# lemerleau/RAFFT

Hardware: AMD Instinct MI355X
Metric: sequences/sec (whole node) on benchmark set, beam N=100; kcal/mol MAE vs CPU (higher is better)
Workload: dtype f32 FFT -> exact int counts, f64 scores, i32 dcal energies

## Files before the change

rafft_amd/csrc/rafft_beam.hip:

```cpp
#pragma once


__device__ inline bool seen_lookup(const uint64_t *tab, uint32_t cap, uint64_t h1, uint64_t h2, uint32_t &free_sl)
{
    const uint32_t mask = cap - 1;
    uint32_t sl = (uint32_t)h1 & mask;
    const ulonglong2 *t2 = (const ulonglong2 *)tab;
    for (;;) {
        const uint32_t s1 = (sl + 1) & mask, s2 = (sl + 2) & mask, s3 = (sl + 3) & mask;
        ulonglong2 e0 = t2[sl], e1 = t2[s1], e2 = t2[s2], e3 = t2[s3];
        pin(e0); pin(e1); pin(e2); pin(e3);
        if (e0.x == 0) { free_sl = sl; return false; }
        if (e0.x == h1 && e0.y == h2) return true;
        if (e1.x == 0) { free_sl = s1; return false; }
        if (e1.x == h1 && e1.y == h2) return true;
        if (e2.x == 0) { free_sl = s2; return false; }
        if (e2.x == h1 && e2.y == h2) return true;
        if (e3.x == 0) { free_sl = s3; return false; }
        if (e3.x == h1 && e3.y == h2) return true;
        sl = (sl + 4) & mask;
    }
}
__device__ inline void seen_insert_at(uint64_t *tab, uint32_t cap, uint64_t h1, uint64_t h2, uint32_t sl)
{
    const uint32_t mask = cap - 1;
    for (;;) {
        unsigned long long old = atomicCAS((unsigned long long *)&tab[2 * (uint64_t)sl], 0ULL, (unsigned long long)h1);
        if (old == 0) { tab[2 * (uint64_t)sl + 1] = h2; return; }
        if (old == h1 && tab[2 * (uint64_t)sl + 1] == h2) return;
        sl = (sl + 1) & mask;
    }
}
__device__ inline bool seen_insert_new(uint64_t *tab, uint32_t cap, uint64_t h1, uint64_t h2)
{
    uint32_t mask = cap - 1, sl = (uint32_t)h1 & mask;
    for (;;) {
        unsigned long long old = atomicCAS((unsigned long long *)&tab[2 * (uint64_t)sl], 0ULL, (unsigned long long)h1);
        if (old == 0) { tab[2 * (uint64_t)sl + 1] = h2; return true; }
        if (old == h1 && tab[2 * (uint64_t)sl + 1] == h2) return false;
        sl = (sl + 1) & mask;
    }
}
__device__ inline void seen_insert(uint64_t *tab, uint32_t cap, uint64_t h1, uint64_t h2)
{
    uint32_t mask = cap - 1, sl = (uint32_t)h1 & mask;
    for (;;) {
        unsigned long long old = atomicCAS((unsigned long long *)&tab[2 * (uint64_t)sl], 0ULL, (unsigned long long)h1);
        if (old == 0) { tab[2 * (uint64_t)sl + 1] = h2; return; }
        if (old == h1 && tab[2 * (uint64_t)sl + 1] == h2) return;
        sl = (sl + 1) & mask;
    }
}


template <int NT>
__device__ inline void seen_rehash(const uint64_t *stab, uint32_t scap, uint64_t *ntab, uint32_t ncap, int tid)
{
    const ulonglong2 *src = (const ulonglong2 *)stab;
    const uint32_t mask = ncap - 1;
    for (uint32_t base = 0; base < scap; base += NT * 4) {
        ulonglong2 e[4];
        unsigned long long old[4];
#pragma unroll
        for (int u = 0; u < 4; u++) { const uint32_t i = base + (uint32_t)u * NT + (uint32_t)tid; e[u] = i < scap ? src[i] : make_ulonglong2(0ULL, 0ULL); }
#pragma unroll
        for (int u = 0; u < 4; u++) { old[u] = 1; if (e[u].x) old[u] = atomicCAS((unsigned long long *)&ntab[2 * (uint64_t)((uint32_t)e[u].x & mask)], 0ULL, (unsigned long long)e[u].x); }
#pragma unroll
        for (int u = 0; u < 4; u++)
            if (e[u].x) {
                if (old[u] == 0) ntab[2 * (uint64_t)((uint32_t)e[u].x & mask) + 1] = e[u].y;
                else seen_insert(ntab, ncap, e[u].x, e[u].y);
            }
    }
}

struct ParentInfo {
    unsigned long long total, cur;
    unsigned long long h1, h2;
    int dcal0, flag;
    int sid, nprod;
    unsigned long long prod;
    int rl0, nrl;
};
static_assert(sizeof(ParentInfo) == 64, "ParentInfo layout");

__device__ __forceinline__ unsigned long long sat_mul(unsigned long long a, unsigned long long b)
{
    const unsigned long long lim = 1ULL << 62;
    if (a == 0 || b == 0) return 0;
    return (a > lim / b) ? lim : a * b;
}

template <int BS_NT>
__global__ __launch_bounds__(BS_NT, BS_NT == 256 ? 5 : 1) void beam_step_kernel(Dev d, int sort_cap)
{
    extern __shared__ __align__(16) unsigned char lds[];
    const size_t r0 = max((size_t)8 * (size_t)sort_cap, (size_t)24 * BS_NT);
    unsigned long long *skey = (unsigned long long *)lds;
    unsigned long long *wk_h1 = (unsigned long long *)lds;
    unsigned long long *wk_h2 = wk_h1 + BS_NT;
    unsigned int *wk_tab = (unsigned int *)(wk_h2 + BS_NT);
    unsigned long long *rl_off = (unsigned long long *)(lds + r0);
    int *rl_cnt = (int *)(rl_off + RL_CAP);
    ParentInfo *pinfo = (ParentInfo *)(rl_cnt + RL_CAP);
    unsigned long long *ppre = (unsigned long long *)(pinfo + d.B);
    int *oldbeam = (int *)(ppre + d.B + 1);
    int *sh = oldbeam + ((d.B + 3) & ~3);
    const int tid = threadIdx.x, lane = tid & 63, wv = tid >> 6;
    const int sq = blockIdx.x;
    if (sq == 0 && tid < NSHARD) d.c->node_prev[tid].v = d.c->node[tid].v;
    if (sq == 0 && tid < NCLS) d.c->n_work[tid].v = 0;
    if (sq == 0) for (int i = tid; i < NCLS * NSHARD; i += BS_NT) d.c->wcur[i / NSHARD][i % NSHARD].v = 0;
    if (sq == 0 && tid < NCLS) d.c->wdone[tid] = 0;
    if (d.done[sq]) return;
    if (tid == 0) sh[27] = d.c->overflow != 0 ? 1 : 0;
    __syncthreads();
    if (sh[27]) return;
    const int nbeam = d.beam_n[sq];
    const int step_no = d.nsteps[sq];
    int *beam = d.beam + (size_t)sq * d.B;
    for (int i = tid; i < nbeam; i += BS_NT) oldbeam[i] = beam[i];
    __syncthreads();

    if (d.traj) {
        if (tid == 0) {
            unsigned long long r = atomicAdd(&d.c->trec_n, 1ULL);
            unsigned long long o = atomicAdd(&d.c->tsid_top, (unsigned long long)nbeam);
            if (r >= d.trec_cap || o + nbeam > d.tsid_cap) { atomicOr(&d.c->overflow, OVF_TRAJ); sh[0] = -1; }
            else { d.trec[r] = make_int4(sq, d.nsteps[sq], nbeam, (int)o); sh[0] = (int)o; }
        }
        __syncthreads();
        int o = sh[0];
        if (o >= 0) for (int i = tid; i < nbeam; i += BS_NT) d.tsid[o + i] = oldbeam[i];
        __syncthreads();
    }
    if (tid == 0) d.nsteps[sq] += 1;

    {
        unsigned long long *istart = ppre;
        int *pnode0 = sh + 32;
        unsigned int irun = 0;
        if (tid == 0) sh[28] = 0;
        __syncthreads();
        for (int b0 = 0; b0 < nbeam; b0 += BS_NT) {
            const int b = b0 + tid;
            int ic = 0;
            if (b < nbeam) {
                const int sid = oldbeam[b];
                StRec r;
                {
                    const uint4 *rp = (const uint4 *)&d.st[sid];
                    uint4 q0 = rp[0], q1 = rp[1], q2 = rp[2], q3 = rp[3], q4 = rp[4], q5 = rp[5], q6 = rp[6];
                    pin(q0); pin(q1); pin(q2); pin(q3); pin(q4); pin(q5); pin(q6);
                    auto u64 = [](unsigned int lo, unsigned int hi) { return (unsigned long long)lo | ((unsigned long long)hi << 32); };
                    r.dcal = (int)q0.y; r.node0 = (int)q0.z; r.nnodes = (int)q0.w; r.nprod = (int)q1.y; r.c0d = (int)q1.z;
                    r.h1 = u64(q2.x, q2.y); r.h2 = u64(q2.z, q2.w); r.cursor = u64(q3.z, q3.w); r.total = u64(q4.z, q4.w);
                    r.prod = u64(q5.x, q5.y); r.c0h1 = u64(q5.z, q5.w); r.c0h2 = u64(q6.x, q6.y);
                }
                ParentInfo pi;
                pi.sid = sid; pi.rl0 = 0; pi.nrl = 0; pi.prod = 0; pi.nprod = 0; pi.total = 0; pi.cur = 0; pi.h1 = 0; pi.h2 = 0; pi.dcal0 = 0;
                if (r.total && r.cursor >= r.total) pi.flag = 1;
                else if (r.total && r.cursor > 0) {
                    pi.flag = 2; pi.total = r.total; pi.cur = r.cursor; pi.h1 = r.c0h1; pi.h2 = r.c0h2; pi.dcal0 = r.c0d;
                    pi.prod = r.prod; pi.nprod = r.nprod; ic = r.nprod;
                } else {
                    pi.flag = 0; pi.total = 1; pi.h1 = r.h1; pi.h2 = r.h2; pi.dcal0 = r.dcal;
                    pnode0[b] = r.node0; ic = r.nnodes;
                    if (ic) atomicAdd(&sh[28], ic);
                }
                pinfo[b] = pi;
            }
            int tot, ex = block_exscan<BS_NT>(ic, sh, &tot);
            if (b < nbeam) istart[b] = irun + (unsigned int)ex;
            irun += (unsigned int)tot;
            __syncthreads();
        }
        const int nitems = (int)irun;
        const int nfirst = sh[28], pshard = (sq + step_no) & (NSHARD - 1);
        unsigned long long pb_raw = 0, pball = 0;
        if (tid == BS_NT - 1 && nfirst) pb_raw = atomicAdd(&d.c->prod[pshard].v, (unsigned long long)nfirst);
        unsigned int run1 = 0, run2 = 0;
        for (int t0 = 0; t0 < nitems; t0 += BS_NT) {
            const int t = t0 + tid;
            int b = -1, i = 0, cnt = 0, cn = -1, first = 0;
            unsigned long long coff = 0;
            if (t < nitems) {
                int lo = 0, hi = nbeam - 1;
                while (lo < hi) { const int mid = (lo + hi + 1) >> 1; if (istart[mid] <= (unsigned long long)t) lo = mid; else hi = mid - 1; }
                b = lo; i = t - (int)istart[b];
                first = pinfo[b].flag == 0 ? 1 : 0;
                if (first) {
                    cn = d.nlist[pnode0[b] + i];
                    if (cn < 0) cn = (int)(((const uint32_t *)d.cslot)[-cn - 1] & 0x7FFFFFFFu) - 1;
                    if (cn >= 0) { cnt = d.nd[cn].ncand; coff = d.nd[cn].cand; }
                    if (cnt > 0) {
                        const Cand *cp = &d.cand[coff];
                        const int dd = cp->ddcal;
                        const ulonglong2 hh = *(const ulonglong2 *)&cp->h1;
                        atomicAdd(&pinfo[b].dcal0, dd);
                        atomicAdd(&pinfo[b].h1, hh.x); atomicAdd(&pinfo[b].h2, hh.y);
                        if (cnt >= 2) {
                            unsigned long long old = pinfo[b].total, seen_;
                            do { seen_ = old; old = atomicCAS(&pinfo[b].total, seen_, sat_mul(seen_, (unsigned long long)cnt)); } while (old != seen_);
                        }
                    }
                } else {
                    const ProdEnt pe = d.prod[pinfo[b].prod + i];
                    cnt = (int)pe.cnt; coff = pe.off; cn = pe.node;
                }
            }
            if (t0 == 0 && tid == BS_NT - 1) {
                unsigned long long v = pb_raw;
                if (v + (unsigned long long)nfirst > d.prod_shard_cap) { atomicOr(&d.c->overflow, OVF_PRODLIST); v = ~0ULL; }
                else v += (unsigned long long)pshard * d.prod_shard_cap;
                *(unsigned long long *)&sh[30] = v;
            }
            const int f1 = (first && cnt > 0) ? 1 : 0, f2 = cnt >= 2 ? 1 : 0;
            int tot12, ex12 = block_exscan<BS_NT>(f1 | (f2 << 16), sh, &tot12);
            if (t0 == 0) pball = *(const unsigned long long *)&sh[30];
            const unsigned int pos1 = run1 + (unsigned int)(ex12 & 0xFFFF), pos2 = run2 + (unsigned int)(ex12 >> 16);
            if (b >= 0) {
                if (i == 0) { pinfo[b].rl0 = (int)pos2; if (first) pinfo[b].prod = pball == ~0ULL ? ~0ULL : pball + pos1; }
                if (f1) {
                    atomicAdd(&pinfo[b].nprod, 1);
                    if (pball != ~0ULL) { ProdEnt pe; pe.cnt = (uint32_t)cnt; pe.node = cn; pe.off = coff; d.prod[pball + pos1] = pe; }
                }
                if (f2) {
                    atomicAdd(&pinfo[b].nrl, 1);
                    if ((int)pos2 < d.rl_cap) { rl_cnt[pos2] = cnt; rl_off[pos2] = coff; }
                }
            }
            run1 += (unsigned int)(tot12 & 0xFFFF); run2 += (unsigned int)(tot12 >> 16);
            __syncthreads();
        }
        for (int b = tid; b < nbeam; b += BS_NT) {
            ParentInfo pi = pinfo[b];
            if (pi.flag == 1) continue;
            if (pi.nrl == 0) pi.rl0 = 0;
            else if (pi.rl0 + pi.nrl > d.rl_cap) pi.rl0 = -1;
            if (pi.flag == 0) {
                if (pi.prod == ~0ULL) { pi.prod = 0; pi.nprod = 0; pi.nrl = 0; pi.rl0 = 0; pi.total = 1; }
                const int np = pi.nprod;
                if (np > d.max_prod) atomicOr(&d.c->overflow, OVF_PROD);
                if (np > 64) atomicMax(&d.c->max_nprod, (unsigned int)np);
                StRec *sr = &d.st[pi.sid];
                sr->prod = pi.prod; sr->nprod = np; sr->c0h1 = pi.h1; sr->c0h2 = pi.h2; sr->c0d = pi.dcal0;
                if (np == 0) { pi.flag = 1; sr->total = 1; sr->cursor = 1; }
            }
            pinfo[b] = pi;
        }
    }
    __syncthreads();

    if (wv == 0) {
        unsigned long long carry = 0;
        const unsigned long long LIM = 1ULL << 63;
        for (int base = 0; base < nbeam; base += 64) {
            const int b = base + lane;
            unsigned long long rem = 0;
            if (b < nbeam && !(pinfo[b].flag & 1)) rem = pinfo[b].total - pinfo[b].cur;
            unsigned long long x = rem;
            for (int o = 1; o < 64; o <<= 1) {
                const unsigned long long y = __shfl_up(x, o, 64);
                if (lane >= o) x = (x > LIM - y) ? LIM : x + y;
            }
            unsigned long long incl = (x > LIM - carry) ? LIM : x + carry;
            if (b < nbeam) ppre[b + 1] = incl;
            carry = __shfl(incl, 63, 64);
        }
        if (lane == 0) ppre[0] = 0;
    }
    for (int i = tid; i < 2 * BS_NT; i += BS_NT) wk_tab[i] = 0;
    __syncthreads();
    uint64_t *stab = d.seen + 2 * d.seen_off[sq];
    uint32_t scap = d.seen_cap[sq], scnt = d.seen_cnt[sq];
    const size_t chb = (size_t)sq * d.ch_cap;
    int nb_branch = 0, nchild = 0;
    int single_from = nbeam;
    if (d.max_branch <= 0) single_from = 0;
    const unsigned long long Ptot = ppre[nbeam];
    unsigned long long W = 0;
    while (single_from == nbeam && W < Ptot) {
        const unsigned long long left = Ptot - W;
        const int chunk = left < (unsigned long long)BS_NT ? (int)left : BS_NT;
        if ((unsigned long long)(scnt + chunk) * 2 > scap) {
            uint32_t ncap = scap;
            while ((unsigned long long)(scnt + BS_NT) * 2 > ncap) ncap <<= 1;
            if (tid == 0) {
                unsigned long long o = atomicAdd(&d.c->seen_top, (unsigned long long)ncap);
                if (o + ncap > d.seen_cap_total) { atomicOr(&d.c->overflow, OVF_SEEN); *(unsigned long long *)&sh[8] = ~0ULL; }
                else *(unsigned long long *)&sh[8] = o;
            }
            __syncthreads();
            unsigned long long o = *(unsigned long long *)&sh[8];
            __syncthreads();
            if (o == ~0ULL) { d.done[sq] = 1; return; }
            uint64_t *ntab = d.seen + 2 * o;
            for (uint32_t i = tid; i < ncap; i += BS_NT) ((ulonglong2 *)ntab)[i] = make_ulonglong2(0ULL, 0ULL);
            __syncthreads();
            seen_rehash<BS_NT>(stab, scap, ntab, ncap, tid);
            __syncthreads();
            stab = ntab; scap = ncap;
            if (tid == 0) { d.seen_off[sq] = o; d.seen_cap[sq] = ncap; }
        }
        const int need = d.max_branch - nb_branch;
        int b = 0, sidb = 0, cd = 0, slot = -1;
        uint32_t free_sl = 0;
        bool cand_new = false, last_combo = false;
        unsigned long long idx = 0, totb = 0, h1 = 0, h2 = 0;
        const unsigned long long pos = W + (unsigned long long)tid;
        if (tid < chunk) {
            int lo = 0, hi = nbeam - 1;
            while (lo < hi) { const int mid = (lo + hi + 1) >> 1; if (ppre[mid] <= pos) lo = mid; else hi = mid - 1; }
            b = lo;
            const ParentInfo pi = pinfo[b];
            sidb = pi.sid; totb = pi.total;
            idx = pi.cur + (pos - ppre[b]);
            last_combo = idx == totb - 1;
            unsigned long long a1 = pi.h1, a2 = pi.h2, rest = idx;
            int ad = pi.dcal0;
            auto divmod = [&](unsigned int c, unsigned int &r) {
                if (rest < (1ULL << 24)) {
                    const unsigned int v = (unsigned int)rest;
                    unsigned int q = (unsigned int)((float)v * __frcp_rn((float)c));
                    int rr = (int)(v - q * c);
                    if (rr < 0) { q--; rr += (int)c; } else if (rr >= (int)c) { q++; rr -= (int)c; }
                    r = (unsigned int)rr; rest = q;
                } else { const unsigned long long q = rest / c; r = (unsigned int)(rest - q * c); rest = q; }
            };
            if (pi.rl0 >= 0) {
                int j = pi.nrl - 1;
                const Cand *const same = d.cand;
                const Cand *pn0 = same, *pn1 = same, *pn2 = same, *pn3 = same, *po0 = same, *po1 = same, *po2 = same, *po3 = same;
                auto next = [&](const Cand *&pn, const Cand *&po) {
                    while (j >= 0 && rest) {
                        unsigned int r;
                        divmod((unsigned int)rl_cnt[pi.rl0 + j], r);
                        j--;
                        if (r) { po = &d.cand[rl_off[pi.rl0 + j + 1]]; pn = po + r; return; }
                    }
                };
                next(pn0, po0); next(pn1, po1); next(pn2, po2); next(pn3, po3);
                {
                    const int dn0 = pn0->ddcal, dn1 = pn1->ddcal, dn2 = pn2->ddcal, dn3 = pn3->ddcal, do0 = po0->ddcal, do1 = po1->ddcal, do2 = po2->ddcal, do3 = po3->ddcal;
                    const ulonglong2 hn0 = *(const ulonglong2 *)&pn0->h1, hn1 = *(const ulonglong2 *)&pn1->h1, hn2 = *(const ulonglong2 *)&pn2->h1, hn3 = *(const ulonglong2 *)&pn3->h1;
                    const ulonglong2 ho0 = *(const ulonglong2 *)&po0->h1, ho1 = *(const ulonglong2 *)&po1->h1, ho2 = *(const ulonglong2 *)&po2->h1, ho3 = *(const ulonglong2 *)&po3->h1;
                    ad += (dn0 - do0) + (dn1 - do1) + (dn2 - do2) + (dn3 - do3);
                    a1 += (hn0.x - ho0.x) + (hn1.x - ho1.x) + (hn2.x - ho2.x) + (hn3.x - ho3.x);
                    a2 += (hn0.y - ho0.y) + (hn1.y - ho1.y) + (hn2.y - ho2.y) + (hn3.y - ho3.y);
                }
                while (j >= 0 && rest) {
                    const Cand *pn = same, *po = same;
                    next(pn, po);
                    ad += pn->ddcal - po->ddcal; a1 += pn->h1 - po->h1; a2 += pn->h2 - po->h2;
                }
            } else {
                for (int j = pi.nprod - 1; j >= 0 && rest; j--) {
                    const ProdEnt pe = d.prod[pi.prod + j];
                    if (pe.cnt < 2) continue;
                    unsigned int r;
                    divmod(pe.cnt, r);
                    if (r) { const Cand *po = &d.cand[pe.off], *pn = po + r; ad += pn->ddcal - po->ddcal; a1 += pn->h1 - po->h1; a2 += pn->h2 - po->h2; }
                }
            }
            h1 = a1 ? a1 : 1; h2 = a2 ? a2 : 1; cd = ad;
            wk_h1[tid] = h1; wk_h2[tid] = h2;
            cand_new = !seen_lookup(stab, scap, h1, h2, free_sl);
        }
        if (cand_new) {
            unsigned int sl = (unsigned int)(h1 ^ (h1 >> 32)) & (2 * BS_NT - 1);
            for (;;) {
                const unsigned int old = atomicCAS(&wk_tab[sl], 0u, (unsigned int)tid + 1u);
                if (old == 0) break;
                if (wk_h1[old - 1] == h1 && wk_h2[old - 1] == h2) { atomicMin(&wk_tab[sl], (unsigned int)tid + 1u); break; }
                sl = (sl + 1) & (2 * BS_NT - 1);
            }
            slot = (int)sl;
        }
        __syncthreads();
        const bool isnew = cand_new && wk_tab[slot < 0 ? 0 : slot] == (unsigned int)tid + 1u;
        const unsigned long long bal = __ballot(isnew);
        if (lane == 0) sh[wv] = __popcll(bal);
        __syncthreads();
        int ex = __popcll(bal & ((1ULL << lane) - 1)), tot = 0;
        for (int w = 0; w < BS_NT / 64; w++) { const int t = sh[w]; if (w < wv) ex += t; tot += t; }
        const bool hit = tot >= need;
        const bool accepted = isnew && ex < need;
        if (accepted) {
            const int ci2 = nchild + ex;
            if (ci2 < d.ch_cap) {
                d.ch_parent[chb + ci2] = (uint16_t)b;
                d.ch_combo[chb + ci2] = idx;
                d.ch_dcal[chb + ci2] = cd;
                d.ch_h[2 * (chb + ci2)] = h1;
                d.ch_h[2 * (chb + ci2) + 1] = h2;
            } else atomicOr(&d.c->overflow, OVF_SORT);
            seen_insert_at(stab, scap, h1, h2, free_sl);
        }
        if (hit) {
            if (accepted && ex == need - 1) {
                sh[21] = b; *(unsigned long long *)&sh[22] = pos;
                d.st[sidb].cursor = idx + 1; d.st[sidb].total = totb;
            }
            __syncthreads();
            const unsigned long long hpos = *(unsigned long long *)&sh[22];
            if (tid < chunk && last_combo && pos < hpos) { d.st[sidb].cursor = totb; d.st[sidb].total = totb; }
            nchild += need; nb_branch += need; scnt += need;
            single_from = sh[21] + 1;
            __syncthreads();
            break;
        }
        if (tid < chunk && last_combo) { d.st[sidb].cursor = totb; d.st[sidb].total = totb; }
        nchild += tot; nb_branch += tot; scnt += tot;
        W += (unsigned long long)chunk;
        for (int i = tid; i < 2 * BS_NT; i += BS_NT) wk_tab[i] = 0;
        __syncthreads();
    }
    if (single_from < nbeam) {
        const int nrest = nbeam - single_from;
        if ((unsigned long long)(scnt + nrest) * 2 > scap) {
            uint32_t ncap = scap;
            while ((unsigned long long)(scnt + nrest + BS_NT) * 2 > ncap) ncap <<= 1;
            if (tid == 0) {
                unsigned long long o = atomicAdd(&d.c->seen_top, (unsigned long long)ncap);
                if (o + ncap > d.seen_cap_total) { atomicOr(&d.c->overflow, OVF_SEEN); *(unsigned long long *)&sh[8] = ~0ULL; }
                else *(unsigned long long *)&sh[8] = o;
            }
            __syncthreads();
            unsigned long long o = *(unsigned long long *)&sh[8];
            __syncthreads();
            if (o == ~0ULL) { d.done[sq] = 1; return; }
            uint64_t *ntab = d.seen + 2 * o;
            for (uint32_t i = tid; i < ncap; i += BS_NT) ((ulonglong2 *)ntab)[i] = make_ulonglong2(0ULL, 0ULL);
            __syncthreads();
            seen_rehash<BS_NT>(stab, scap, ntab, ncap, tid);
            __syncthreads();
            stab = ntab; scap = ncap;
            if (tid == 0) { d.seen_off[sq] = o; d.seen_cap[sq] = ncap; }
        }
        for (int base = single_from; base < nbeam; base += BS_NT) {
            const int b = base + tid;
            int isnew = 0;
            uint32_t free_sl = 0;
            uint64_t h1 = 0, h2 = 0;
            if (b < nbeam && pinfo[b].flag == 0) {
                h1 = pinfo[b].h1; h2 = pinfo[b].h2;
                if (h1 == 0) h1 = 1;
                if (h2 == 0) h2 = 1;
                isnew = seen_lookup(stab, scap, h1, h2, free_sl) ? 0 : 1;
                for (int e = single_from; isnew && e < b; e++)
                    if (pinfo[e].flag == 0) {
                        uint64_t g1 = pinfo[e].h1, g2 = pinfo[e].h2;
                        if (g1 == 0) g1 = 1;
                        if (g2 == 0) g2 = 1;
                        if (g1 == h1 && g2 == h2) isnew = 0;
                    }
            }
            int tot, ex = block_exscan_flag<BS_NT>(isnew, sh, &tot);
            if (isnew) {
                const int ci2 = nchild + ex;
                if (ci2 < d.ch_cap) {
                    d.ch_parent[chb + ci2] = (uint16_t)b;
                    d.ch_combo[chb + ci2] = 0;
                    d.ch_dcal[chb + ci2] = pinfo[b].dcal0;
                    d.ch_h[2 * (chb + ci2)] = h1;
                    d.ch_h[2 * (chb + ci2) + 1] = h2;
                } else atomicOr(&d.c->overflow, OVF_SORT);
                seen_insert_at(stab, scap, h1, h2, free_sl);
            }
            if (b < nbeam && pinfo[b].flag == 0) { d.st[oldbeam[b]].cursor = 1; d.st[oldbeam[b]].total = pinfo[b].total; }
            nchild += tot; nb_branch += tot; scnt += tot;
            __syncthreads();
        }
    }
    if (tid == 0) { d.seen_cnt[sq] = scnt; atomicAdd(&d.c->xstat[1][sq & (NSHARD - 1)].children, (unsigned long long)nchild); }
    if (nchild > d.ch_cap) nchild = d.ch_cap;

    const int N = nchild + nbeam;
    if (N > sort_cap) { if (tid == 0) atomicOr(&d.c->overflow, OVF_SORT); d.done[sq] = 1; return; }
    for (int i = tid; i < N; i += BS_NT) {
        unsigned long long key;
        if (i < nchild) key = ((unsigned long long)(uint32_t)(d.ch_dcal[chb + i] + 0x40000000) << 32) | (uint32_t)i;
        else key = ((unsigned long long)(uint32_t)(d.st[oldbeam[i - nchild]].dcal + 0x40000000) << 32) | (uint32_t)i;
        skey[i] = key;
    }
    __syncthreads();
    {
        const int K = N < d.B ? N : d.B;
        select_smallest_inplace<BS_NT>(skey, N, K, rl_cnt, sh);
        if (K <= RL_CAP) {
            unsigned long long *outk = rl_off;
            for (int i = tid; i < K; i += BS_NT) {
                const unsigned long long ki = skey[i];
                int r = 0;
                for (int j = 0; j < K; j++) r += skey[j] < ki ? 1 : 0;
                outk[r] = ki;
            }
            __syncthreads();
            for (int i = tid; i < K; i += BS_NT) skey[i] = outk[i];
            __syncthreads();
        } else {
        int M = 2; while (M < K) M <<= 1;
        for (int i = K + tid; i < M; i += BS_NT) skey[i] = ~0ULL;
        __syncthreads();
        for (int k2 = 2; k2 <= M; k2 <<= 1)
            for (int j = k2 >> 1; j > 0; j >>= 1) {
                for (int i = tid; i < M; i += BS_NT) {
                    int ixj = i ^ j;
                    if (ixj > i) {
                        unsigned long long a = skey[i], bb = skey[ixj];
                        bool up = (i & k2) == 0;
                        if (up ? a > bb : a < bb) { skey[i] = bb; skey[ixj] = a; }
                    }
                }
                __syncthreads();
            }
        }
    }
    const int nnew = N < d.B ? N : d.B;
    int nsurv_child = 0;
    for (int base = 0; base < nnew; base += BS_NT) {
        int i = base + tid, f = 0;
        if (i < nnew) f = ((uint32_t)skey[i] < (uint32_t)nchild) ? 1 : 0;
        int tot, ex = block_exscan_flag<BS_NT>(f, sh, &tot);
        (void)ex;
        nsurv_child += tot;
        __syncthreads();
    }
    if (nsurv_child == 0) {
        if (tid == 0) {
            d.done[sq] = 1;
            atomicAdd(&d.c->n_done, 1u);
            if (!d.traj) {
                unsigned long long r = atomicAdd(&d.c->trec_n, 1ULL);
                unsigned long long o = atomicAdd(&d.c->tsid_top, (unsigned long long)nbeam);
                if (r >= d.trec_cap || o + nbeam > d.tsid_cap) atomicOr(&d.c->overflow, OVF_TRAJ);
                else {
                    d.trec[r] = make_int4(sq, 0, nbeam, (int)o);
                    for (int i = 0; i < nbeam; i++) d.tsid[o + i] = oldbeam[i];
                }
            }
        }
        return;
    }
    if (tid == 0) {
        unsigned long long sb = atomicAdd(&d.c->n_struct, (unsigned long long)nsurv_child);
        unsigned int mb = atomicAdd(&d.c->n_mat, (unsigned int)nsurv_child);
        atomicAdd(&d.c->xstat[1][sq & (NSHARD - 1)].struct_len, (unsigned long long)nsurv_child * (unsigned long long)d.seq_len[sq]);
        if (sb + nsurv_child > d.st_cap || mb + nsurv_child > d.mat_cap) { atomicOr(&d.c->overflow, OVF_STRUCT); sh[24] = -1; }
        else { sh[24] = (int)sb; sh[25] = (int)mb; }
    }
    __syncthreads();
    const int sbase = sh[24], mbase = sh[25];
    __syncthreads();
    if (sbase < 0) { d.done[sq] = 1; return; }
    int run = 0;
    const int Lsq = d.seq_len[sq];
    const unsigned long long soff_sq = (unsigned long long)d.seq_off[sq];
    for (int base = 0; base < nnew; base += BS_NT) {
        int i = base + tid, f = 0;
        uint32_t ord = 0;
        if (i < nnew) { ord = (uint32_t)skey[i]; f = (ord < (uint32_t)nchild) ? 1 : 0; }
        int c_dcal = 0;
        unsigned int c_par = 0;
        unsigned long long c_combo = 0;
        ulonglong2 c_h = make_ulonglong2(0ULL, 0ULL);
        if (f) {
            const size_t c = chb + ord;
            c_dcal = d.ch_dcal[c]; c_par = d.ch_parent[c]; c_combo = d.ch_combo[c]; c_h = *(const ulonglong2 *)&d.ch_h[2 * c];
        }
        int tot, ex = block_exscan_flag<BS_NT>(f, sh, &tot);
        if (i < nnew) {
            if (f) {
                pin(c_dcal); pin(c_par); pin(c_combo); pin(c_h);
                const int sid = sbase + run + ex;
                const ParentInfo &pp_ = pinfo[c_par];
                StRec *sr = &d.st[sid];
                sr->seq = sq; sr->dcal = c_dcal; sr->h1 = c_h.x; sr->h2 = c_h.y; sr->parent = oldbeam[c_par]; sr->combo = c_combo;
                sr->cursor = 0; sr->total = 0; sr->nnodes = 0;
                MatRec mr;
                mr.sid = sid; mr.sq = sq; mr.L = Lsq; mr.dcal = c_dcal; mr.nprod = pp_.nprod; mr.pad = 0;
                mr.combo = c_combo; mr.prod = pp_.prod; mr.soff = soff_sq;
                d.mat[mbase + run + ex] = mr;
                beam[i] = sid;
            } else
                beam[i] = oldbeam[ord - nchild];
        }
        run += tot;
        __syncthreads();
    }
    if (tid == 0) d.beam_n[sq] = nnew;
}
```

rafft_amd/csrc/rafft_config.h:

```cpp
#pragma once
#include <cstdio>
#include <cstdlib>
#include <cstring>

struct Config {
    double reserve_frac = 0.10;
    double est = 0.0;
    long linger_us = 600;
    long spin_us = 200, nap_us = 50;
    double big_wave_frac = 0.10;
    int cls1_p = 512;
    int c3_direct = 1;
    int c3_switch = -1;
    int direct_n = 1024;
    int force_fft = 0;
    int prod = 1;
    int no_memo = 0;
    int small_n4 = 16, small_n5 = 32;
    int small_wg = 4;
    int slab = 64;
    int fetch = 4, taper = 25;
    int mat_tile = 64;
    int rl_cap = -1;
    int wide_below = 600;
    int merge_below = -1;
    int merge2_below = -1;
    int split = -1;
    int serial = 0;
    int trace = 0;
    int spans = -1;
    int max_waves = 3;
    int merge_seqs = 16384;
    int trace_alloc = 0;
    int test_hard_fail = -1;
    int test_max_prod = 0;
    int test_ovf_at = -1;
    int seen_fixed = 0;
    int test_cand_limit = 0;
};
static_assert(sizeof(Config) == 8 * 6 + 4 * 30, "Config: 8-byte fields first, an even number of ints - no padding (same_config compares bytes)");

inline Config read_config()
{
    Config c;
    auto I = [](const char *name, int &v) { if (const char *e = getenv(name)) v = atoi(e); };
    auto L = [](const char *name, long &v) { if (const char *e = getenv(name)) v = atol(e); };
    auto F = [](const char *name, double &v) { if (const char *e = getenv(name)) v = atof(e); };
    auto B = [](const char *name, int &v) { if (getenv(name)) v = 1; };
    I("RAFFT_CLS1_P", c.cls1_p); I("RAFFT_C3_DIRECT", c.c3_direct); I("RAFFT_C3_SWITCH", c.c3_switch); I("RAFFT_DIRECT_N", c.direct_n);
    I("RAFFT_FORCE_FFT", c.force_fft); I("RAFFT_PROD", c.prod); I("RAFFT_NO_MEMO", c.no_memo);
    if (const char *e = getenv("RAFFT_SMALL")) { int a = 16, b = 32; if (sscanf(e, "%d,%d", &a, &b) >= 1) { c.small_n4 = a; c.small_n5 = b; } }
    I("RAFFT_SMALL_WG", c.small_wg); I("RAFFT_SLAB", c.slab); I("RAFFT_FETCH", c.fetch); I("RAFFT_TAPER", c.taper);
    I("RAFFT_WIDE_BELOW", c.wide_below); I("RAFFT_MERGE_BELOW", c.merge_below); I("RAFFT_MERGE2_BELOW", c.merge2_below);
    F("RAFFT_RESERVE_FRAC", c.reserve_frac); I("RAFFT_SPLIT", c.split); I("RAFFT_SERIAL", c.serial);
    I("RAFFT_TRACE", c.trace); if (getenv("RAFFT_TRACE") && c.trace < 1) c.trace = 1;
    I("RAFFT_SPANS", c.spans);
    I("RAFFT_MAX_WAVES", c.max_waves); I("RAFFT_MERGE_SEQS", c.merge_seqs);
    L("RAFFT_LINGER_US", c.linger_us); L("RAFFT_SCHED_SPIN_US", c.spin_us); L("RAFFT_SCHED_NAP_US", c.nap_us); F("RAFFT_BIG_WAVE_FRAC", c.big_wave_frac);
    B("RAFFT_TRACE_ALLOC", c.trace_alloc);
#ifndef RAFFT_NO_TEST_HOOKS
    I("RAFFT_MAT_TILE", c.mat_tile); I("RAFFT_RL_CAP", c.rl_cap); F("RAFFT_EST", c.est); I("RAFFT_SEEN_FIXED", c.seen_fixed);
    I("RAFFT_TEST_CAND_LIMIT", c.test_cand_limit); I("RAFFT_TEST_HARD_FAIL", c.test_hard_fail); I("RAFFT_TEST_MAX_PROD", c.test_max_prod); I("RAFFT_TEST_OVF_AT", c.test_ovf_at);
#endif
    return c;
}
inline bool same_config(const Config &a, const Config &b) { return memcmp(&a, &b, sizeof(Config)) == 0; }
```

rafft_amd/csrc/rafft_host_ctx.h:

```cpp
#pragma once

namespace {

thread_local std::string g_err;
int fail(int code, const std::string &msg)
{
    g_err = msg;
    return code;
}

#define HIPCHK(x)                                                                                      \
    do {                                                                                               \
        hipError_t e_ = (x);                                                                           \
        if (e_ != hipSuccess)                                                                          \
            return fail(RAFFT_ERR_HIP, std::string(#x) + ": " + hipGetErrorString(e_));                 \
    } while (0)

struct Buf {
    void *p = nullptr;
    size_t cap = 0;
};
struct PinBuf { void *p = nullptr; size_t cap = 0; };

#define MAX_PIPES 4
#define WS_BUFFERS(X)                                                                                                           \
    X(codes, 1) X(seq_off, 1) X(seq_len, 1) X(beam, 1) X(beam_n, 1) X(done, 1) X(nsteps, 1) X(ch_parent, 1) X(ch_combo, 1)      \
    X(ch_dcal, 1) X(ch_h, 1) X(seen, 1) X(seen_off, 1) X(seen_cap, 1) X(seen_cnt, 1) X(st, 1) X(prod, 1) X(nd, 1) X(nlist, 1)   \
    X(nd_slot, 1) X(cslot, 1) X(pos, 1) X(br, 1) X(sp, 1) X(cand, 1) X(looptab, 1) X(trec, 1) X(tsid, 1) X(work0, 1)            \
    X(work1, 1) X(work2, 1) X(work3, 1) X(work4, 1) X(work5, 1) X(mat, 1) X(counters, 1) X(row_off, 1) X(out_db, 1)             \
    X(out_dcal, 1) X(row_off2, 1) X(out_db2, 1) X(out_dcal2, 1) X(dbg, 0) X(big, 0)
struct Workspace {
    bool ready = false;
    hipStream_t stream = nullptr;
    hipStream_t cls_stream[NCLS] = {};
    hipStream_t copy_stream = nullptr;
    hipEvent_t ev_fork = nullptr, ev_join[NCLS] = {}, ev_hot = nullptr, ev_copy = nullptr;
    void *hot = nullptr;
#define X(name, matched) Buf name;
    WS_BUFFERS(X)
#undef X
    template <class F> static void for_each_buf(F f)
    {
#define X(name, matched) f(&Workspace::name, matched != 0);
        WS_BUFFERS(X)
#undef X
    }
    int match(const Workspace &o);
    void release_buffers()
    {
        for_each_buf([&](Buf Workspace::*m, bool) {
            Buf &b = this->*m;
            if (b.p) { hipError_t e_ = hipFree(b.p); (void)e_; b.p = nullptr; b.cap = 0; }
        });
    }
    size_t bytes() const
    {
        size_t t = 0;
        for_each_buf([&](Buf Workspace::*m, bool) { t += (this->*m).cap; });
        return t;
    }
};

struct Ctx {
    bool ready = false;
    int device = -1;
    int n_cu = 256;
    EnergyTables *T = nullptr;
    double T_temp = -1e300;
    bool T_dirty = true;
    rafft_par::ParamSet *P = nullptr;
    float2 *tw = nullptr;
    size_t hbm_total = 0;
    Workspace ws[MAX_PIPES];
    std::vector<PinBuf> pin_free;
    std::mutex pin_mu;
    std::vector<hipEvent_t> ev_free;
    std::vector<void *> garbage;
    std::mutex gc_mu;
    std::mutex ws_mu;
    rafft_stats stats{};
    std::mutex mu;
    std::mutex qmu;
    std::condition_variable qcv_sched, qcv_done;
    std::deque<std::shared_ptr<struct Batch>> submitted;
    int n_inflight = 0;
    bool last_submit_async = false;
    std::chrono::steady_clock::time_point t_last_submit{};
    Config proc_cfg;
    Config sched_cfg;
    bool sched_started = false;
    bool stop = false;
    std::thread sched_thread;
};
Ctx &g = *new Ctx();

std::atomic<unsigned long long> g_dev_allocs{0}, g_dev_bytes{0}, g_dev_worst_us{0}, g_pin_allocs{0}, g_pin_bytes{0};

int ensure(Buf &b, size_t bytes, bool exact = false)
{
    if (bytes <= b.cap) return 0;
    const auto t0_ = std::chrono::steady_clock::now();
    const size_t old_cap = b.cap;
    if (b.p) { std::lock_guard<std::mutex> lk(g.gc_mu); g.garbage.push_back(b.p); b.p = nullptr; b.cap = 0; }
    size_t want = exact ? bytes : bytes + std::min<size_t>(bytes / (old_cap ? 2 : 8), (size_t)256 << 20) + 256;
    want = (want + ((size_t)2 << 20) - 1) & ~(((size_t)2 << 20) - 1);
    hipError_t e = hipMalloc(&b.p, want);
    if (e != hipSuccess) {
        (void)hipGetLastError();
        std::vector<void *> junk;
        { std::lock_guard<std::mutex> lk(g.gc_mu); junk.swap(g.garbage); }
        for (void *q : junk) { hipError_t e2 = hipFree(q); (void)e2; }
        want = (bytes + 256 + ((size_t)2 << 20) - 1) & ~(((size_t)2 << 20) - 1);
        e = hipMalloc(&b.p, want);
    }
    {
        const unsigned long long us = (unsigned long long)std::chrono::duration_cast<std::chrono::microseconds>(std::chrono::steady_clock::now() - t0_).count();
        g_dev_allocs++; g_dev_bytes += want;
        unsigned long long w = g_dev_worst_us.load();
        while (us > w && !g_dev_worst_us.compare_exchange_weak(w, us)) { }
    }
    if (g.proc_cfg.trace_alloc) fprintf(stderr, "[rafft] ptr %p (mod 2MiB %zu KiB) ", b.p, ((size_t)(uintptr_t)b.p & (((size_t)2 << 20) - 1)) >> 10);
    if (g.proc_cfg.trace_alloc) fprintf(stderr, "[rafft] t=%.3f device buffer -> %.1f MB in %.3f ms\n", std::chrono::duration<double>(std::chrono::steady_clock::now().time_since_epoch()).count(), (double)want / 1e6, std::chrono::duration<double, std::milli>(std::chrono::steady_clock::now() - t0_).count());
    if (e != hipSuccess) {
        b.p = nullptr;
        return fail(RAFFT_ERR_HIP, std::string("hipMalloc(") + std::to_string(want) + "): " + hipGetErrorString(e));
    }
    b.cap = want;
    return 0;
}

int Workspace::match(const Workspace &o)
{
    int rc = 0;
    for_each_buf([&](Buf Workspace::*m, bool matched) { if (matched && !rc) rc = ensure(this->*m, (o.*m).cap, true); });
    return rc;
}

rafft_par::ParamSet &param_set()
{
    if (!g.P) { g.P = new rafft_par::ParamSet(); rafft_par::builtin(*g.P); }
    return *g.P;
}

int ensure_tables(double temp)
{
    if (!g.T_dirty && g.T_temp == temp) return 0;
    std::unique_ptr<EnergyTables> h(new EnergyTables());
    std::string err;
    if (!rafft_par::scaled_tables(param_set(), temp, h.get(), err)) return fail(RAFFT_ERR_TEMP, err);
    HIPCHK(hipMemcpy(g.T, h.get(), sizeof(EnergyTables), hipMemcpyHostToDevice));
    g.T_temp = temp; g.T_dirty = false;
    return 0;
}

int init_ws(Workspace &w)
{
    if (w.ready) return 0;
    int plo = 0, phi = 0;
    HIPCHK(hipDeviceGetStreamPriorityRange(&plo, &phi));
    const int idx = (int)(&w - g.ws);
    const int prio = idx == 1 ? phi : idx == 3 ? plo : 0;
    HIPCHK(hipStreamCreateWithPriority(&w.stream, hipStreamNonBlocking, prio));
    for (int c = 0; c < NCLS; c++) {
        HIPCHK(hipStreamCreateWithPriority(&w.cls_stream[c], hipStreamNonBlocking, prio));
        HIPCHK(hipEventCreateWithFlags(&w.ev_join[c], hipEventDisableTiming));
    }
    HIPCHK(hipStreamCreateWithFlags(&w.copy_stream, hipStreamNonBlocking));
    HIPCHK(hipEventCreateWithFlags(&w.ev_fork, hipEventDisableTiming));
    HIPCHK(hipEventCreateWithFlags(&w.ev_copy, hipEventDisableTiming));
    HIPCHK(hipEventCreateWithFlags(&w.ev_hot, hipEventDisableTiming | hipEventBlockingSync));
    static_assert(offsetof(Counters, node) <= 1024, "hot counters must fit the pinned read-back slot");
    HIPCHK(hipHostMalloc(&w.hot, 1024, hipHostMallocDefault));
    w.ready = true;
    return 0;
}

int init_ctx(int device)
{
    if (g.ready && (device < 0 || device == g.device)) {
        HIPCHK(hipSetDevice(g.device));
        return 0;
    }
    g.proc_cfg = read_config();
    int ndev = 0;
    hipError_t e = hipGetDeviceCount(&ndev);
    if (e != hipSuccess || ndev == 0)
        return fail(RAFFT_ERR_NO_DEVICE, "no HIP device: libraffthip.so has no CPU fallback");
    if (device < 0) device = 0;
    if (device >= ndev) return fail(RAFFT_ERR_NO_DEVICE, "device ordinal out of range");
    if (g.ready) return fail(RAFFT_ERR_PARAM, "library already initialised on another device in this process");
    HIPCHK(hipSetDevice(device));
    hipDeviceProp_t prop;
    HIPCHK(hipGetDeviceProperties(&prop, device));
    g.hbm_total = prop.totalGlobalMem;
    g.n_cu = prop.multiProcessorCount > 0 ? prop.multiProcessorCount : 256;
    HIPCHK(hipMalloc((void **)&g.T, sizeof(EnergyTables)));
    g.T_dirty = true;
    std::vector<float2> tw(MAX_P / 2);
    for (int m = 0; m < MAX_P / 2; m++) {
        double a = -2.0 * M_PI * (double)m / (double)MAX_P;
        tw[m] = make_float2((float)cos(a), (float)sin(a));
    }
    HIPCHK(hipMalloc((void **)&g.tw, sizeof(float2) * tw.size()));
    HIPCHK(hipMemcpy(g.tw, tw.data(), sizeof(float2) * tw.size(), hipMemcpyHostToDevice));
    g.device = device;
    g.ready = true;
    return init_ws(g.ws[0]);
}

static void free_garbage()
{
    std::vector<void *> junk;
    { std::lock_guard<std::mutex> lk(g.gc_mu); junk.swap(g.garbage); }
    for (void *p : junk) { hipError_t e_ = hipFree(p); (void)e_; }
}

PinBuf pin_acquire(size_t bytes)
{
    std::lock_guard<std::mutex> lk(g.pin_mu);
    size_t want = 256 * 1024;
    while (want < bytes) want <<= 1;
    int best = -1;
    for (size_t i = 0; i < g.pin_free.size(); i++)
        if (g.pin_free[i].cap >= bytes && g.pin_free[i].cap <= 4 * want && (best < 0 || g.pin_free[i].cap < g.pin_free[best].cap)) best = (int)i;
    if (best >= 0) { PinBuf b = g.pin_free[best]; g.pin_free.erase(g.pin_free.begin() + best); return b; }
    PinBuf b;
    const auto t0_ = std::chrono::steady_clock::now();
    if (hipHostMalloc(&b.p, want, hipHostMallocDefault) != hipSuccess) { b.p = nullptr; return b; }
    g_pin_allocs++; g_pin_bytes += want;
    if (g.proc_cfg.trace_alloc) fprintf(stderr, "[rafft] t=%.3f pinned chunk %.1f MB in %.3f ms (pool %zu)\n", std::chrono::duration<double>(std::chrono::steady_clock::now().time_since_epoch()).count(), (double)want / 1e6, std::chrono::duration<double, std::milli>(std::chrono::steady_clock::now() - t0_).count(), g.pin_free.size());
    b.cap = want;
    return b;
}
void pin_release(PinBuf b)
{
    if (!b.p) return;
    std::lock_guard<std::mutex> lk(g.pin_mu);
    size_t held = 0;
    for (auto &x : g.pin_free) held += x.cap;
    if (g.pin_free.size() < 64 && held + b.cap <= ((size_t)4 << 30)) g.pin_free.push_back(b);
    else {
        const auto t0_ = std::chrono::steady_clock::now();
        hipError_t e = hipHostFree(b.p); (void)e;
        if (g.proc_cfg.trace_alloc) fprintf(stderr, "[rafft] pinned chunk freed in %.3f ms\n", std::chrono::duration<double, std::milli>(std::chrono::steady_clock::now() - t0_).count());
    }
}

struct PinChunk {
    PinBuf b;
    explicit PinChunk(PinBuf x) : b(x) {}
    ~PinChunk() { pin_release(b); }
    PinChunk(const PinChunk &) = delete;
    PinChunk &operator=(const PinChunk &) = delete;
};

}
```

rafft_amd/csrc/rafft_io_kernels.hip:

```cpp
#pragma once


struct StageIn { const uint32_t *src[8]; uint32_t *dst[8]; unsigned long long words[8]; int n; };
__global__ __launch_bounds__(256) void stage_in_kernel(StageIn si)
{
    for (int k = 0; k < si.n; k++) {
        const uint32_t *src = si.src[k];
        uint32_t *dst = si.dst[k];
        for (unsigned long long i = (unsigned long long)blockIdx.x * 256 + threadIdx.x; i < si.words[k]; i += (unsigned long long)gridDim.x * 256) dst[i] = src[i];
    }
}

__global__ void init_roots_kernel(Dev d)
{
    const int sq = blockIdx.x, tid = threadIdx.x;
    const int L = d.seq_len[sq];
    const unsigned long long off = (unsigned long long)d.seq_off[sq];
    for (int x = tid; x < L; x += blockDim.x) d.pos[off + x] = (uint16_t)(d.pos_packed ? x | (d.codes[off + x] << 12) : x);

    if (tid == 0) {
        d.st[sq].seq = sq; d.st[sq].dcal = 0; d.st[sq].h1 = 0; d.st[sq].h2 = 0;
        d.st[sq].sp = 0; d.st[sq].nsp = 0; d.st[sq].node0 = sq; d.st[sq].nnodes = L > 0 ? 1 : 0; d.st[sq].cursor = 0; d.st[sq].total = 0;
        d.st[sq].parent = -1; d.st[sq].combo = 0;
        d.nd[sq].seq = sq; d.nd[sq].pdcal = 0; d.nd[sq].pos = off; d.nd[sq].n = L; d.nd[sq].ci = -1; d.nd[sq].cj = L;
        d.nd[sq].L = L; d.nd[sq].soff = off;
        d.nd[sq].br = 0; d.nd[sq].nbr = 0; d.nlist[sq] = sq;
        d.nd[sq].ncand = -1; d.nd[sq].cand = 0;
        d.beam[(size_t)sq * d.B] = sq; d.beam_n[sq] = 1; d.nsteps[sq] = 0;
        d.done[sq] = L > 0 ? 0 : 1;
        d.seen_cnt[sq] = 0;
        if (L > 0) {
            int cls = node_class(L, L, 0, 0, d.cls1_P, d.cls1_br);
            unsigned int w = atomicAdd(&d.c->n_work[cls].v, 1u);
            d.work[cls][w] = sq;
        }
    }
}


struct OutRec { long long off; int row0, w, cnt, L; };
__global__ void output_kernel(Dev d, int nrows, int nrec, const OutRec *recs, char *out_db, int *out_dcal)
{
    extern __shared__ __align__(16) uint8_t out_row[];
    for (int r = blockIdx.x; r < nrows; r += gridDim.x) {
        int lo = 0, hi = nrec - 1;
        while (lo < hi) { const int mid = (lo + hi + 1) >> 1; if (recs[mid].row0 <= r) lo = mid; else hi = mid - 1; }
        const OutRec rc = recs[lo];
        const int k = r - rc.row0;
        const int sid = d.tsid[rc.w + k];
        const int L = rc.L;
        for (int x = threadIdx.x; x < L; x += blockDim.x) out_row[x] = '.';
        __syncthreads();
        int s = sid, par = -1, np = 0;
        unsigned long long spo = 0;
        if (s >= 0) { par = d.st[s].parent; np = d.st[s].nsp; spo = d.st[s].sp; }
        while (s >= 0) {
            const int s2 = par;
            int par2 = -1, np2 = 0;
            unsigned long long spo2 = 0;
            if (s2 >= 0) { par2 = d.st[s2].parent; np2 = d.st[s2].nsp; spo2 = d.st[s2].sp; }
            const uint32_t *pl = d.sp + spo;
            for (int x = threadIdx.x; x < np; x += blockDim.x) { const uint32_t u = pl[x]; out_row[u & 0xFFFFu] = '('; out_row[u >> 16] = ')'; }
            s = s2; par = par2; np = np2; spo = spo2;
        }
        __syncthreads();
        char *o = out_db + rc.off + (long long)k * (L + 1);
        for (int x = threadIdx.x; x < L; x += blockDim.x) o[x] = (char)out_row[x];
        if (threadIdx.x == 0) { o[L] = 0; out_dcal[r] = d.st[sid].dcal; }
        __syncthreads();
    }
}


__global__ __launch_bounds__(64) void eval_kernel(const EnergyTables *ET, int n, const uint8_t *codes, const int16_t *pts,
                                                  const long long *off, const int *len, int *out, int *status, int *guessed)
{
    const int s = blockIdx.x, lane = threadIdx.x;
    if (s >= n) return;
    const int L = len[s];
    const uint8_t *S = codes + off[s];
    PlainView pv{pts + off[s]};
    const SmallT *T = &ET->s;
    const BigT *B = &ET->b;
    int e = 0, bad = 0;
    if (lane == 0) e += loop_energy(T, B, S, L, pv, -1, L, &bad);
    for (int i = lane; i < L; i += 64) {
        int j = pv(i);
        if (j > i) e += loop_energy(T, B, S, L, pv, i, j, &bad);
    }
    for (int o = 32; o > 0; o >>= 1) { e += __shfl_xor(e, o, 64); bad |= __shfl_xor(bad, o, 64); }
    if (lane == 0) { out[s] = e; status[s] = (bad & 1) ? 8 : 0; if (guessed) guessed[s] = (bad >> 1) & 1; }
}
```

rafft_amd/csrc/rafft_kernels.h:

```cpp
#pragma once
#include "rafft_device.h"

struct alignas(16) Cand {
    int32_t ddcal;
    uint16_t mi, mj, nb, cut_hi;
    uint32_t cut_lo;
    uint64_t h1, h2;
    __host__ __device__ void set_cuts(int lo0, int hi0, int loo, int hio)
    {
        const unsigned long long v = (unsigned long long)lo0 | ((unsigned long long)hi0 << 12) | ((unsigned long long)loo << 24) | ((unsigned long long)hio << 36);
        cut_lo = (uint32_t)v; cut_hi = (uint16_t)(v >> 32);
    }
    __host__ __device__ void get_cuts(int &lo0, int &hi0, int &loo, int &hio) const
    {
        const unsigned long long v = (unsigned long long)cut_lo | ((unsigned long long)cut_hi << 32);
        lo0 = (int)(v & 4095); hi0 = (int)((v >> 12) & 4095); loo = (int)((v >> 24) & 4095); hio = (int)((v >> 36) & 4095);
    }
};
static_assert(sizeof(Cand) == 32, "Cand must be 32 bytes");

#define NSHARD 64
#ifndef SEEN0
#define SEEN0 8192
#endif
#define NCLS 6
#define NGEN 4
struct ShardCtr { unsigned long long v; unsigned long long pad[7]; };

struct alignas(128) StRec {
    int32_t seq, dcal, node0, nnodes, parent, nprod;
    int32_t c0d, nsp;
    uint64_t h1, h2;
    uint64_t sp, cursor, combo, total, prod;
    uint64_t c0h1, c0h2;
    uint64_t pad2[3];
};
static_assert(sizeof(StRec) == 128, "StRec is two cache lines");

struct alignas(64) NodeRec {
    int32_t seq, pdcal, n, ci, cj, nbr, ncand, L;
    uint64_t pos, br, cand, soff;
};
static_assert(sizeof(NodeRec) == 64, "NodeRec must be one cache line");

struct ProdEnt { uint32_t cnt; int32_t node; uint64_t off; };
struct alignas(16) MatRec { int32_t sid, sq, L, dcal, nprod, pad; uint64_t combo, prod, soff; };

struct Counters {
    unsigned int n_mat;
    unsigned int overflow;
    unsigned int n_done;
    unsigned int max_nprod;
    unsigned int pad0_[12];
    unsigned long long n_struct, pad1_[7];
    unsigned long long trec_n, tsid_top, pad2_[6];
    unsigned long long seen_top, pad3_[7];
    struct WorkCtr { unsigned int v; unsigned int pad[15]; } n_work[NCLS];
    unsigned long long n_expand, sum_n, sum_lags, n_children, sum_struct_len, n_alias, sum_nbr;
    unsigned long long cls_items[NCLS], cls_sum_n[NCLS], cls_sum_lags[NCLS];
    ShardCtr node[NSHARD], pos[NSHARD], br[NSHARD], sp[NSHARD], cand[NSHARD], node_prev[NSHARD], prod[NSHARD];
    ShardCtr nlist[NSHARD];
    ShardCtr wcur[NCLS][NSHARD];
    unsigned long long wdone[NCLS];
    unsigned long long wdone_pad[8 - NCLS];
    struct StatLine { unsigned long long items, n, lags, nbr, alias, children, struct_len, evals, guessed, kept_guessed, pad[6]; } xstat[NCLS][NSHARD];
};

enum { OVF_STRUCT = 1, OVF_NODE = 2, OVF_POS = 4, OVF_SP = 8, OVF_CAND = 16, OVF_SEEN = 32,
       OVF_TRAJ = 64, OVF_WORK = 128, OVF_PROD = 256, OVF_SORT = 512, OVF_BR = 1024, OVF_LOOPTAB = 2048, OVF_PRODLIST = 4096 };

struct DebugOut {
    int *n_ranked, *lag, *nb, *mi, *mj, *ddcal, *kept;
    double *corval, *score;
};

struct Dev {
    const EnergyTables *T;
    const float2 *tw;
    int S;
    const uint8_t *codes;
    const int *seq_off, *seq_len;
    int K, B, max_branch, min_hp, traj, memo, force_fft, rl_cap, mat_tile, merge_cls;
    double *big_keyv; size_t big_stride;
    int max_prod;
    int fetch_bulk, taper_pct;
    int direct_n;
    int sm_n4, sm_n5;
    int cand_slab;
    int cls1_P, cls1_br;
    int c3_switch;
    double min_nrj, gc, au, gu;
    int *beam, *beam_n, *done, *nsteps;
    int ch_cap;
    uint16_t *ch_parent; uint64_t *ch_combo; int *ch_dcal; uint64_t *ch_h;
    uint64_t *seen; uint64_t seen_cap_total;
    uint64_t *seen_off; uint32_t *seen_cap, *seen_cnt;
    uint32_t st_cap;
    StRec *st;
    ProdEnt *prod; uint64_t prod_shard_cap;
    uint32_t nd_cap;
    uint64_t nd_base, nd_shard_cap, pos_base, pos_shard_cap, br_shard_cap, sp_shard_cap, cand_shard_cap;
    NodeRec *nd;
    int *nlist;
    unsigned long long *cslot;
    uint32_t *nd_slot;
    unsigned long long *looptab; uint64_t looptab_cap;
    uint16_t *pos; uint64_t pos_cap;
    int pos_packed;
    uint32_t *br; uint64_t br_cap;
    uint32_t *sp; uint64_t sp_cap;
    Cand *cand; uint64_t cand_cap;
    int4 *trec; uint32_t trec_cap;
    int *tsid; uint64_t tsid_cap;
    int *work[NCLS]; uint32_t work_cap;
    MatRec *mat; uint32_t mat_cap;
    Counters *c;
    DebugOut dbg;
};

#define CLS0_P 4096
#define CLS1_P 512
#define CLS01_L 1280
#define CLS1_BR 256
#define CLS2_P 2048
#define MAX_P 8192
#define MAX_BR 1024
#define BIG_BR 4095
#define BIG_N 32768
#define LDS_SEQ 4096
#define MAX_PROD 64
#define MAX_PROD_LONG 1024
#define RL_CAP 1024

__host__ __device__ inline int next_pow2_ge(int x) { int p = 2; while (p < x) p <<= 1; return p; }
#define SM_SPAN 448
__host__ __device__ inline int node_class(int n, int span, int nbr, int merge_cls = 0, int cls1_P = CLS1_P, int cls1_br = CLS1_BR,
                                          int K = 0, int sm_n4 = 0, int sm_n5 = 0)
{
    if (merge_cls == 0 && n >= 2 && n <= sm_n5 && 2 * n - 1 <= K && span <= SM_SPAN) {
        if (n <= sm_n4 && nbr <= 16) return 4;
        if (sm_n5 > sm_n4 && nbr <= 32) return 5;
    }
    int P = next_pow2_ge(2 * n - 1);
    if (P > MAX_P || nbr > MAX_BR) return 0;
    if (merge_cls == 3) return 3;
    if (merge_cls == 2) return P <= CLS2_P ? 2 : 3;
    if (span <= CLS01_L && P <= cls1_P && nbr <= cls1_br) return 1;
    if (P <= CLS2_P) return 2;
    return 3;
}

#define MASK_F_WORDS 5
#define MASK_WORDS 10
struct ExpandLds {
    int offA, szA, off_pos, off_code, off_p2, off_S, off_br, off_rk, off_nb, off_mi, off_mj, off_dd, off_keep, off_w, off_misc,
        per_team,
        off_tab, off_tw,
        total;
};
__host__ __device__ inline ExpandLds expand_lds(int Pmax, int Lmax, int nmax, int brmax, int Kmax, bool tab_lds, int wpb = 1, bool nofft = false, int nt = 512,
                                                bool code_lds = true)
{
    ExpandLds l;
    auto al = [](int x) { return (x + 15) & ~15; };
    l.offA = 0;
    l.szA = al(16 * Pmax);
    if (nofft) {
        const int need1 = 8 * Pmax + 8 * MASK_WORDS * ((nmax + 63) / 64) + 8 + (nt > 64 && 24 * nt > 1152 ? 24 * nt : 1152) , need2 = 8 * Pmax + 10 * (brmax + 1) + 16, need3 = 8 * Pmax + 8 * Kmax + 64;
        l.szA = al(need1 > need2 ? (need1 > need3 ? need1 : need3) : (need2 > need3 ? need2 : need3));
    }
    int o = l.szA;
    l.off_pos = o; o += al(2 * nmax + 2);
    l.off_code = o; if (code_lds) o += al(nmax);
    l.off_p2 = o; if (code_lds) o += al(4 * ((nmax + 15) / 16 + 1));
    l.off_S = o; o += al(Lmax + 8);
    l.off_br = o; o += al(4 * brmax);
    const int lag_bytes = al(2 * next_pow2_ge(Kmax)) + 4 * al(2 * Kmax) + al(4 * Kmax);
    const bool lag_in_A = Pmax == MAX_P && Kmax > 256 && 8 * Pmax + 24 * 1024 + lag_bytes <= l.szA;
    int oa = lag_in_A ? 8 * Pmax + 24 * 1024 : 0;
    int &q = lag_in_A ? oa : o;
    l.off_rk = q; q += al(2 * next_pow2_ge(Kmax));
    l.off_nb = q; q += al(2 * Kmax);
    l.off_mi = q; q += al(2 * Kmax);
    l.off_mj = q; q += al(2 * Kmax);
    l.off_dd = q; q += al(4 * Kmax);
    l.off_keep = q; q += al(2 * Kmax);
    l.off_w = o; if (!nofft) o += al(25 * 8);
    l.off_misc = o; o += 128;
    l.per_team = o;
    int sh = 0;
    l.off_tab = sh; if (tab_lds) sh += al((int)sizeof(SmallT));
    l.off_tw = sh; if (tab_lds && Pmax <= CLS2_P && !nofft) sh += al(8 * (Pmax / 2));
    l.total = wpb * l.per_team + sh;
    return l;
}
```

rafft_amd/csrc/rafft_plan.h:

```cpp
#pragma once

namespace {

struct ClsCfg { int nt, Pmax, Lmax, nmax, brmax, Kmax, lds, grid; int wpb; bool nofft; bool direct3 = false; };

static int cls1_P(const Config &cfg) { return std::max(256, std::min(next_pow2_ge(cfg.cls1_p), CLS1_P)); }
static int cls1_br(const Config &cfg) { return std::min(CLS1_BR, (8 * cls1_P(cfg) - 16) / 10 - 1); }

int class_cfg(const Config &cfg, int K, int maxL, ClsCfg out[NGEN + 1], bool nofft1 = false, bool nofft2 = false, bool direct3_ok = false)
{
    const bool longseq = maxL > LDS_SEQ;
    const int P[NGEN] = {CLS0_P, cls1_P(cfg), CLS2_P, MAX_P}, LM[NGEN] = {0, CLS01_L, longseq ? 0 : LDS_SEQ, longseq ? 0 : LDS_SEQ};
    const int NT[NGEN] = {512, 64, 256, 512}, BR[NGEN] = {BIG_BR + 1, nofft1 ? 128 : cls1_br(cfg), MAX_BR, MAX_BR};
    int wpb1 = nofft1 ? 16 : 12;
    {
        const int Kmax1 = std::max(1, std::min(K, cls1_P(cfg) - 1));
        if (wpb1 == 16 && expand_lds(cls1_P(cfg), CLS01_L, cls1_P(cfg) / 2, BR[1], Kmax1, true, wpb1, nofft1, 64).total > 160 * 1024) wpb1 = 12;
        if (expand_lds(cls1_P(cfg), CLS01_L, cls1_P(cfg) / 2, BR[1], Kmax1, true, wpb1, nofft1, 64).total > 160 * 1024) wpb1 = 1;
    }
    const int WPB[NGEN] = {1, wpb1, 1, 1};
    const bool TAB[NGEN] = {false, WPB[1] > 1, false, false};
    for (int c = 0; c < NGEN; c++) {
        const int big_n = maxL > 16384 ? BIG_N : 16384;
        int nmax = c == 0 ? big_n : P[c] / 2;
        int Kmax = std::max(1, std::min(K, c == 0 ? 2 * big_n - 1 : P[c] - 1));
        const bool nf = (c == 1 && nofft1 && WPB[1] > 1) || (c == 2 && nofft2);
        ExpandLds l = expand_lds(P[c], LM[c], nmax, BR[c], Kmax, TAB[c], WPB[c], nf, NT[c], c != 0);
        const int ws_parts = maxL > 16384 ? 8 * std::max(Kmax, 1) : std::max(std::min(8 * std::max(Kmax, 1), NT[c]), Kmax);
        if (c == 0 && longseq && (8 * MASK_WORDS * (big_n / 64) + 24 * ws_parts + 4096 > 16 * P[c] || 10 * (BR[c] + 1) + 16 + 24 * Kmax + 2048 > 16 * P[c]))
            return fail(RAFFT_ERR_PARAM, std::string("nb_mode too large for the LDS scratch of the class for regions beyond 4096 positions: with a sequence of ") +
                                         (maxL > 16384 ? "more than 16384 nt it must stay at or below 106" : "more than 4096 nt it must stay below ~400") +
                                         " (this wave: nb_mode " + std::to_string(K) + ", longest sequence " + std::to_string(maxL) + " nt)");
        if (c >= 1 && (10 * (BR[c] + 1) + 16 > 8 * P[c] || 2 * P[c] + 1152 + 16 > 8 * P[c] || (NT[c] > 64 && NT[c] * 24 > 8 * P[c])))
            return fail(RAFFT_ERR_PARAM, "internal: expand LDS plan does not fit its size class");
        if (c >= 1 && LM[c] > 0 && l.off_S < LDS_SEQ)
            return fail(RAFFT_ERR_PARAM, "internal: the LDS copy of the bases sits too low for its shifted pointer");
        const int per_cu = std::max(1, std::min(32 / (NT[c] / 64), WPB[c] * ((160 * 1024) / l.total)));
        out[c] = {NT[c], P[c], LM[c], nmax, BR[c], Kmax, l.total, g.n_cu * per_cu, WPB[c], nf};
        const bool reachable = c == 0 ? longseq : (c < 3 || maxL > CLS2_P / 2);
        if (l.total > 160 * 1024 && reachable)
            return fail(RAFFT_ERR_PARAM, "nb_mode too large for the LDS-resident expand kernel: it must stay below 2048 (below ~400 when a "
                                         "sequence is longer than 4096 nt)");
        if (l.total > 160 * 1024) out[c].lds = 160 * 1024, out[c].Kmax = 1;
    }
    const int c3_direct = cfg.c3_direct;
    if (c3_direct && direct3_ok && !longseq) {
        const int Kmax = std::max(1, std::min(K, MAX_P - 1)), nmax = MAX_P / 2, Pd = 2048;
        const int Cc = std::max(1, std::min(8, 256 / std::max(Kmax, 1)));
        const bool fits = 8 * MASK_WORDS * (nmax / 64) + 24 * Cc * Kmax + 2048 + 64 <= 16 * Pd && 10 * (MAX_BR + 1) + 16 + 8 * Kmax + 2048 <= 16 * Pd;
        ExpandLds l = expand_lds(Pd, 0, nmax, MAX_BR, Kmax, false, 1, false, 256);
        if (fits && l.total <= 80 * 1024) {
            const int per_cu = std::max(1, std::min(3, (160 * 1024) / l.total));
            out[NGEN] = out[3];
            out[3] = {256, Pd, 0, nmax, MAX_BR, Kmax, l.total, g.n_cu * per_cu, 1, false, true};
        }
    }
    return 0;
}

template <int NT, bool TAB, int WPB = 1, int LONGSEQ = 0, int PROD = 0>
int launch_expand(const Dev &d, int cls, const ClsCfg &cf, unsigned n_teams, hipStream_t st)
{
    static int lds_set = 0;
    if (cf.lds > lds_set) {
        HIPCHK(hipFuncSetAttribute((const void *)expand_kernel<NT, TAB, WPB, LONGSEQ, PROD>, hipFuncAttributeMaxDynamicSharedMemorySize, cf.lds));
        lds_set = cf.lds;
    }
    const unsigned n_blocks = (n_teams + WPB - 1) / WPB;
    hipLaunchKernelGGL((expand_kernel<NT, TAB, WPB, LONGSEQ, PROD>), dim3(n_blocks), dim3(NT * WPB), cf.lds, st, d, cls, cf.Pmax, cf.Lmax, cf.nmax, cf.brmax, cf.Kmax);
    HIPCHK(hipGetLastError());
    return 0;
}

int launch_expand_cls(const Config &cfg, const Dev &d, int cls, const ClsCfg cf[NGEN + 1], unsigned n_blocks, hipStream_t st)
{
    const bool prod_ok = cfg.prod != 0;
    if (cls >= NGEN) {
        const bool prod = prod_ok && d.dbg.lag == nullptr;
        if (cls == 4 && prod) hipLaunchKernelGGL((expand_small_kernel<16, true>), dim3(n_blocks), dim3(64 * SM_WG_WAVES), small_lds_bytes<16>(), st, d, cls);
        else if (cls == 4) hipLaunchKernelGGL((expand_small_kernel<16, false>), dim3(n_blocks), dim3(64 * SM_WG_WAVES), small_lds_bytes<16>(), st, d, cls);
        else if (prod) hipLaunchKernelGGL((expand_small_kernel<32, true>), dim3(n_blocks), dim3(64 * SM_WG_WAVES), small_lds_bytes<32>(), st, d, cls);
        else hipLaunchKernelGGL((expand_small_kernel<32, false>), dim3(n_blocks), dim3(64 * SM_WG_WAVES), small_lds_bytes<32>(), st, d, cls);
        HIPCHK(hipGetLastError());
        return 0;
    }
    const bool longseq = cf[2].Lmax == 0;
    const int nf = cf[cls].nofft ? 0x2000 : 0;
    const bool nodiag = prod_ok && d.dbg.lag == nullptr && !d.force_fft && d.gc >= 0.0 && d.au >= 0.0 && d.gu >= 0.0;
    const bool prod = nodiag && nf;
    if (cls == 0) return nodiag ? launch_expand<512, false, 1, 2, 2>(d, 0, cf[0], n_blocks, st) : launch_expand<512, false, 1, 2>(d, 0, cf[0], n_blocks, st);
    if (longseq && cls == 2) return prod ? launch_expand<256, false, 1, 1, 1>(d, 2 | nf, cf[2], n_blocks, st) : launch_expand<256, false, 1, 1>(d, 2 | nf, cf[2], n_blocks, st);
    if (longseq && cls == 3) return nodiag && !nf ? launch_expand<512, false, 1, 1, 2>(d, 3, cf[3], n_blocks, st) : launch_expand<512, false, 1, 1>(d, 3 | nf, cf[3], n_blocks, st);
    if (cls == 1) {
        if (cf[1].wpb == 16 && prod) return launch_expand<64, true, 16, 0, 1>(d, 1 | nf, cf[1], n_blocks, st);
        if (cf[1].wpb == 16) return launch_expand<64, true, 16>(d, 1 | nf, cf[1], n_blocks, st);
        if (cf[1].wpb == 12) return launch_expand<64, true, 12>(d, 1 | nf, cf[1], n_blocks, st);
        return launch_expand<64, false>(d, 1, cf[1], n_blocks, st);
    }
    if (cls == 2) return prod ? launch_expand<256, false, 1, 0, 1>(d, 2 | nf, cf[2], n_blocks, st) : launch_expand<256, false>(d, 2 | nf, cf[2], n_blocks, st);
    if (cf[3].direct3) {
        if (int rc = nodiag ? launch_expand<256, false, 1, 2, 3>(d, 3 | 0x8000, cf[3], n_blocks, st) : launch_expand<256, false, 1, 2>(d, 3 | 0x8000, cf[3], n_blocks, st)) return rc;
        const unsigned nb_fft = std::min<unsigned>(n_blocks, (unsigned)cf[NGEN].grid);
        return nodiag ? launch_expand<512, false, 1, 0, 2>(d, 3 | 0x4000, cf[NGEN], nb_fft, st) : launch_expand<512, false>(d, 3 | 0x4000, cf[NGEN], nb_fft, st);
    }
    return nodiag ? launch_expand<512, false, 1, 0, 2>(d, 3, cf[3], n_blocks, st) : launch_expand<512, false>(d, 3, cf[3], n_blocks, st);
}

struct Caps {
    size_t st, nd, pos, br, sp, cand, seen, trec, tsid, work, mat, looptab;
    int ch_cap, sort_cap;
    size_t bytes;
    bool capped;
};

static uint32_t seen_slots0(int L, const rafft_params &p, const Config &cfg)
{
    if (cfg.seen_fixed) return SEEN0;
    const double l = (double)L;
    const double e = l <= 130 ? 26.0 * l : l <= 300 ? 3380.0 + 13.0 * (l - 130) : l <= 500 ? 5590.0 + 10.5 * (l - 300) : l <= 1000 ? 7690.0 + 2.4 * (l - 500) : 8890.0 + 5.6 * (l - 1000);
    const double per_step = p.max_branch > 0 ? std::min((double)p.max_branch, 8.2 * (double)p.max_stack) : (double)p.max_stack;
    const double need = 2.0 * (e * std::max(per_step / 410.0, 0.1) + 384.0);
    uint32_t cap = 2048;
    while ((double)cap < need && cap < (1u << 22)) cap <<= 1;
    return cap;
}
static size_t seen_slots0_wave(const int *len, size_t S, const rafft_params &p, const Config &cfg, size_t budget_slots, uint32_t *out)
{
    uint32_t limit = 1u << 22;
    for (;;) {
        size_t tot = 0;
        for (size_t i = 0; i < S; i++) { const uint32_t c = std::min(seen_slots0(len[i], p, cfg), limit); if (out) out[i] = c; tot += c; }
        if (tot <= budget_slots || limit <= SEEN0) return tot;
        limit >>= 1;
    }
}
#define SEEN0_BUDGET ((size_t)192 << 20)

Caps plan_caps(const Config &cfg, size_t S, size_t sumL, const rafft_params &p, double est, double seen0_per_seq)
{
    Caps c;
    const size_t B = (size_t)p.max_stack;
    double avgL = S ? (double)sumL / (double)S : 1.0;
    double nstruct = (double)S * (1.0 + (double)B * est);
    c.st = (size_t)std::min(nstruct, 2.0e9) + 64;
    double nodes_per = avgL / 60.0 + 4.0;
    c.nd = (size_t)std::min((double)c.st * nodes_per, 2.0e9) + 64;
    c.capped = nstruct > 2.0e9 || (double)c.st * nodes_per > 2.0e9;
    c.pos = (size_t)((double)sumL + (double)(c.st - S) * avgL * 0.9) + 4096;
    c.br = c.nd * 3 + 4096;
    c.sp = (size_t)((double)(c.st - S) * (avgL * 0.05 + 24.0)) + 4096;
    c.cand = c.nd * (size_t)std::min(std::max(p.nb_mode, 1), 8) + 4096;
    const bool memo_on = p.min_nrj == 0.0 && !cfg.no_memo;
    if (memo_on) c.cand = std::min(c.cand, (size_t)((double)c.st * (60.0 + avgL / 40.0)) + 4096);
    c.cand = std::max<size_t>(c.cand, (size_t)NSHARD * 16384);
    size_t cand_limit = ((size_t)1 << 30) - 4096;
    if (cfg.test_cand_limit > 0) cand_limit = std::min<size_t>(cand_limit, std::max<size_t>((size_t)cfg.test_cand_limit, (size_t)NSHARD * 16384));
    if (c.cand > cand_limit) { c.cand = cand_limit; c.capped = true; }
    double per_seq_seen = std::min(std::max(std::max(5.0 * est * ((double)B + (double)p.max_branch / 4.0), seen0_per_seq), 16384.0), 16777216.0);
    c.seen = (size_t)((double)S * seen0_per_seq) + std::max((size_t)((double)S * per_seq_seen), (size_t)4 << 20);
    c.trec = p.traj ? S * (size_t)(est * 3 + 16) : S + 16;
    c.tsid = c.trec * B + 16;
    c.mat = S * B + 16;
    c.nd = std::max<size_t>(c.nd, S + (size_t)NSHARD * 2048);
    c.pos = std::max<size_t>(c.pos, sumL + (size_t)NSHARD * (16 * (size_t)avgL + 4096));
    c.sp = std::max<size_t>(c.sp, (size_t)NSHARD * (2 * (size_t)avgL + 4096));
    c.br = std::max<size_t>(c.br, (size_t)NSHARD * 8192);
    c.work = c.nd;
    c.looptab = 1024; while (c.looptab < c.nd) c.looptab <<= 1;
    c.ch_cap = p.max_branch + p.max_stack + 8;
    int need = p.max_branch + 2 * p.max_stack + 8;
    int m2 = 2; while (m2 < p.max_stack) m2 <<= 1;
    c.sort_cap = std::max((need + 1) & ~1, m2);
    c.bytes = c.st * 128 + c.nd * (64 + 4 + 4 + 6 * 4 + 16) + c.pos * 2 + c.br * 4 + c.sp * 4 + c.cand * (32 + 8) + c.seen * 16 +
              c.looptab * 8 + c.trec * 16 + c.tsid * 4 + c.mat * 48 + S * (size_t)c.ch_cap * 32 + S * B * 4;
    return c;
}

static size_t merge_cap()
{
    return (size_t)std::max(1, g.sched_cfg.merge_seqs);
}

struct JobPlan { Caps caps; std::vector<uint32_t> seen_cap0; size_t seen0_total; double seen0_avg; };
JobPlan plan_job(const Config &cfg, const rafft_params &p, const std::vector<SeqIn> &seqs, double est)
{
    JobPlan jp;
    const size_t S = seqs.size();
    std::vector<int> len(S);
    size_t sumL = 0;
    for (size_t i = 0; i < S; i++) { len[i] = seqs[i].len; sumL += (size_t)seqs[i].len; }
    jp.seen_cap0.resize(S);
    jp.seen0_total = seen_slots0_wave(len.data(), S, p, cfg, SEEN0_BUDGET, jp.seen_cap0.data());
    jp.seen0_avg = (double)jp.seen0_total / (double)std::max<size_t>(S, 1);
    jp.caps = plan_caps(cfg, S, sumL, p, est, jp.seen0_avg);
    return jp;
}

}
```

rafft_amd/csrc/rafft_wave.h:

```cpp
#pragma once

namespace {

hipEvent_t next_event(std::vector<hipEvent_t> &used)
{
    hipEvent_t e = nullptr;
    if (!g.ev_free.empty()) { e = g.ev_free.back(); g.ev_free.pop_back(); }
    else if (hipEventCreate(&e) != hipSuccess) return nullptr;
    used.push_back(e);
    return e;
}

struct Span { hipEvent_t a, b; int kind; };
static int g_span_level = 1;
static inline bool span_on(int kind) { return g_span_level >= 2 || (g_span_level == 1 && kind == 11); }
#define SPAN_REC(ev, st, kind) do { if (span_on(kind)) HIPCHK(hipEventRecord((ev), (st))); } while (0)

struct HostOut {
    std::vector<rafft_seq_result> seq;
    std::vector<std::vector<int>> step_size, step_off;
    std::vector<int> one_size, one_off;
    std::vector<const char *> db_ptr;
    std::vector<const int *> dcal_ptr;
    std::vector<std::shared_ptr<struct PinChunk>> chunks;
    rafft_result res;
    void resize(int n) { seq.resize(n); step_size.resize(n); step_off.resize(n); one_size.assign(n, 0); one_off.assign(n, 0); dcal_ptr.assign(n, nullptr); db_ptr.assign(n, nullptr); }
};
void free_out(HostOut *o) { delete o; }

struct Batch;
struct Job { std::vector<SeqIn> seqs; double est; int depth; std::vector<std::shared_ptr<Batch>> members; bool no_merge = false;
             bool big_prod = false; };

struct Batch {
    rafft_params p;
    Config cfg;
    int n_seq = 0;
    std::vector<char> seqbuf;
    std::vector<uint8_t> codebuf;
    HostOut *ho = nullptr;
    std::deque<Job> lane[2];
    int pending = 0;
    int rc = 0;
    std::string err;
    std::vector<Span> spans;
    std::vector<hipEvent_t> events;
    rafft_stats stats{};
    std::chrono::steady_clock::time_point t0;
    bool done = false;
};

struct SeamIn {
    DebugOut dbg;
    std::vector<uint16_t> pos;
    std::vector<uint32_t> br;
    int ci, cj, pdcal;
};

struct HostTimer {
    double &a;
    std::chrono::steady_clock::time_point t = std::chrono::steady_clock::now();
    ~HostTimer() { a += std::chrono::duration<double, std::milli>(std::chrono::steady_clock::now() - t).count(); }
};

struct Wave {
    Workspace &ws;
    const Config &cfg;
    rafft_params p;
    std::vector<SeqIn> seqs;
    double est;
    std::vector<std::shared_ptr<Batch>> members;
    Batch &bt;
    std::vector<Span> &spans;
    const SeamIn *seam;
    size_t S = 0, sumL = 0, B = 0, bs_lds[2] = {0, 0}, mat_lds = RAFFT_MAX_LEN, out_row_lds = RAFFT_MAX_LEN;
    double reserve = 1.0;
    bool longseq = false;
    std::vector<int> off, len;
    std::vector<uint32_t> seen_cap0;
    size_t seen0_total = 0;
    ClsCfg cf[NGEN + 1];
    Caps c;
    Dev d;
    Counters hc;
    unsigned n_active = 0, ovf = 0, last_mat = 0;
    int merged_now = 0, merge_target = 0;
    int steps = 0;
    int depth = 0;
    bool big_prod = false, want_big_prod = false;
    bool finished = false;
    long long last_rows_bytes = 0;
    std::vector<OutRec> early_recs, late_recs;
    PinBuf stage{};
    bool draining = false;
    struct Tail { double ms_loop = 0, stats = 0, gather = 0; std::chrono::steady_clock::time_point t0; } tail;
    ~Wave() { pin_release(stage); }
    size_t harvested = 0;
    int emit_rows(size_t first, size_t count, bool early, double *t_gather);
    int result = 0;
    std::chrono::steady_clock::time_point tw0, tw1;
    double ms_setup = 0, ms_issue = 0, ms_after = 0;

    Wave(Workspace &w, std::vector<std::shared_ptr<Batch>> m, std::vector<SeqIn> s, double e, const SeamIn *sm = nullptr)
        : ws(w), cfg(m[0]->cfg), p(m[0]->p), seqs(std::move(s)), est(e), members(std::move(m)), bt(*members[0]), spans(members[0]->spans), seam(sm) {}
    HostOut &out_of(int local_seq) { return *members[seqs[local_seq].bi]->ho; }

    double since(std::chrono::steady_clock::time_point t) const
    {
        return std::chrono::duration<double, std::milli>(std::chrono::steady_clock::now() - t).count();
    }
    hipEvent_t next_event() { return ::next_event(bt.events); }
    bool heavy(unsigned below) const { return S >= 256 && !finished && (steps < 3 || last_mat >= below); }
    int setup();
    int issue_step();
    int ready()
    {
        const hipError_t e = hipEventQuery(ws.ev_hot);
        if (e == hipSuccess) return 1;
        if (e == hipErrorNotReady) return 0;
        fail(RAFFT_ERR_HIP, std::string("hipEventQuery: ") + hipGetErrorString(e));
        return -1;
    }
    std::chrono::steady_clock::time_point t_issued;
    int after_beam();
    int issue_materialize(unsigned n_mat);
    int finish() { const int rc = finish_body(); if (rc) { finished = true; draining = false; if (!result) result = rc; } return rc; }
    int finish_done() { const int rc = finish_done_body(); if (rc) { finished = true; if (!result) result = rc; } return rc; }
    int finish_body();
    int finish_done_body();
};

int Wave::setup()
{
    S = seqs.size();
    tw0 = std::chrono::steady_clock::now();
    if (cfg.test_hard_fail >= 0 && (int)S == cfg.test_hard_fail) return fail(RAFFT_ERR_PARAM, "test hook: hard failure of this wave");
    off.resize(S); len.resize(S);
    sumL = 0;
    for (size_t i = 0; i < S; i++) { off[i] = (int)sumL; len[i] = seqs[i].len; sumL += seqs[i].len; }
    const size_t st_codes = 0, st_off = (sumL + 16 + 63) & ~(size_t)63, st_len = st_off + ((S * 4 + 63) & ~(size_t)63),
                 st_ctr = st_len + ((S * 4 + 63) & ~(size_t)63), st_soff = st_ctr + ((sizeof(Counters) + 63) & ~(size_t)63),
                 st_scap = st_soff + ((S * 8 + 63) & ~(size_t)63), st_bytes = st_scap + S * 4;
    stage = pin_acquire(st_bytes);
    if (!stage.p) return fail(RAFFT_ERR_HIP, "hipHostMalloc failed for the input staging buffer");
    uint8_t *codes = (uint8_t *)stage.p + st_codes;
    for (size_t i = 0; i < S; i++) {
        uint8_t *dst = codes + off[i];
        if (seqs[i].c) memcpy(dst, seqs[i].c, (size_t)seqs[i].len);
        else {
            const unsigned char *src = (const unsigned char *)seqs[i].s;
            for (int x = 0; x < seqs[i].len; x++) dst[x] = kBaseCode[src[x]] & 7;
        }
    }
    memset(codes + sumL, 0, 16);
    memcpy((char *)stage.p + st_off, off.data(), S * 4);
    memcpy((char *)stage.p + st_len, len.data(), S * 4);
    const double ms_enc = since(tw0);
    int maxL = 0;
    for (size_t i = 0; i < S; i++) maxL = std::max(maxL, len[i]);
    const int direct_n_ = cfg.direct_n;
    const bool force_fft_ = cfg.force_fft != 0;
    const bool nofft1 = !seam && !force_fft_ && direct_n_ >= cls1_P(cfg) / 2 && p.gc_wei >= 0.0 && p.au_wei >= 0.0 && p.gu_wei >= 0.0;
    const bool nofft2 = nofft1 && direct_n_ >= CLS2_P / 2;
    if (int rc = class_cfg(cfg, p.nb_mode, maxL, cf, nofft1, nofft2, nofft1)) return rc;
    if (cfg.trace)
        for (int c = 0; c < NGEN; c++)
            fprintf(stderr, "[rafft] expand class %d: %d threads x %d regions per workgroup, P <= %d, branches <= %d, lags <= %d, LDS %d B%s\n", c, cf[c].nt, cf[c].wpb,
                    cf[c].Pmax, cf[c].brmax, cf[c].Kmax, cf[c].lds, cf[c].nofft ? " (no FFT buffers)" : "");
    merge_target = maxL > CLS2_P / 2 ? 3 : 2;
    JobPlan jp = plan_job(cfg, p, seqs, est);
    seen_cap0 = std::move(jp.seen_cap0);
    seen0_total = jp.seen0_total;
    const double seen0_avg = jp.seen0_avg;
    c = jp.caps;
    if (std::max((size_t)c.sort_cap * 8, (size_t)24 * 1024) + RL_CAP * 12 + (size_t)(p.max_stack + 4) * (sizeof(ParentInfo) + 16) + 1024 > 150 * 1024)
        return fail(RAFFT_ERR_PARAM, "max_branch + 2*max_stack too large for the LDS-resident beam sort");
    B = (size_t)p.max_stack;

    size_t Sr = S;
    Caps cr = c;
    if (S < merge_cap() && !seam) {
        const double reserve_frac = cfg.reserve_frac;
        const size_t tries[2] = {S >= 256 ? merge_cap() : std::max<size_t>(S, std::min<size_t>(64, 32 * S)), S >= 256 ? std::min(merge_cap(), 5 * S) : S};
        Sr = S;
        for (size_t want : tries) {
            if (want <= S) continue;
            Caps big = plan_caps(cfg, want, (size_t)((double)sumL * (double)want / (double)S), p, est, seen0_avg);
            if (big.bytes <= (size_t)((double)g.hbm_total * reserve_frac)) { cr = big; Sr = want; break; }
        }
    }
    reserve = (double)Sr / (double)S;
    const size_t sumLr = Sr == S ? sumL : (size_t)((double)sumL * (double)Sr / (double)S);
#define ENS(buf, bytes) do { if (int rc_ = ensure(ws.buf, (bytes))) return rc_; } while (0)
    ENS(codes, sumLr + 16); ENS(seq_off, Sr * 4); ENS(seq_len, Sr * 4);
    ENS(beam, Sr * B * 4); ENS(beam_n, Sr * 4); ENS(done, Sr * 4); ENS(nsteps, Sr * 4);
    ENS(ch_parent, Sr * c.ch_cap * 2); ENS(ch_combo, Sr * c.ch_cap * 8); ENS(ch_dcal, Sr * c.ch_cap * 4); ENS(ch_h, Sr * c.ch_cap * 16);
    ENS(seen, cr.seen * 16); ENS(seen_off, Sr * 8); ENS(seen_cap, Sr * 4); ENS(seen_cnt, Sr * 4);
    ENS(st, cr.st * sizeof(StRec)); ENS(prod, cr.nd * 16);
    ENS(nd, cr.nd * sizeof(NodeRec)); ENS(nlist, cr.nd * 4); ENS(nd_slot, cr.nd * 4); ENS(cslot, cr.cand * 8);
    ENS(pos, cr.pos * 2); ENS(br, cr.br * 4); ENS(sp, cr.sp * 4); ENS(cand, cr.cand * 32);
    ENS(looptab, cr.looptab * 8);
    ENS(trec, cr.trec * 16); ENS(tsid, cr.tsid * 4);
    ENS(work0, cr.work * 4); ENS(work1, cr.work * 4); ENS(work2, cr.work * 4); ENS(work3, cr.work * 4); ENS(work4, cr.work * 4); ENS(work5, cr.work * 4);
    ENS(mat, cr.mat * sizeof(MatRec));
    ENS(counters, sizeof(Counters));
#undef ENS


    memset(&d, 0, sizeof d);
    d.T = g.T; d.tw = g.tw; d.S = (int)S;
    d.codes = (const uint8_t *)ws.codes.p; d.seq_off = (const int *)ws.seq_off.p; d.seq_len = (const int *)ws.seq_len.p;
    d.K = p.nb_mode; d.B = p.max_stack; d.max_branch = p.max_branch; d.min_hp = p.min_hp; d.traj = p.traj;
    d.min_nrj = p.min_nrj; d.gc = p.gc_wei; d.au = p.au_wei; d.gu = p.gu_wei;
    d.memo = (p.min_nrj == 0.0) ? 1 : 0;
    if (cfg.no_memo) d.memo = 0;
    if (cfg.force_fft) d.force_fft = 1;
    d.rl_cap = RL_CAP;
    longseq = maxL > LDS_SEQ;
    d.pos_packed = longseq ? 0 : 1;
    d.max_prod = (longseq || big_prod) ? MAX_PROD_LONG : MAX_PROD;
    if (cfg.test_max_prod > 0 && !big_prod && !longseq) d.max_prod = std::max(1, std::min(cfg.test_max_prod, MAX_PROD));
    if (longseq) {
        d.big_stride = (size_t)2 * cf[0].nmax + (size_t)2 * cf[0].nmax / 4;
        if (int rc = ensure(ws.big, (size_t)cf[0].grid * d.big_stride * 8)) return rc;
        d.big_keyv = (double *)ws.big.p;
    } else if (cf[3].direct3) {
        d.big_stride = (size_t)MAX_P + (size_t)MAX_P / 4;
        if (int rc = ensure(ws.big, (size_t)cf[3].grid * d.big_stride * 8)) return rc;
        d.big_keyv = (double *)ws.big.p;
    }
    d.cls1_P = cls1_P(cfg); d.cls1_br = cf[1].brmax;
    d.c3_switch = cfg.c3_switch >= 0 ? cfg.c3_switch : g.n_cu;
    d.cand_slab = std::max(16, cfg.slab);
    d.fetch_bulk = std::max(1, cfg.fetch);
    d.taper_pct = std::max(0, std::min(100, cfg.taper));
    d.direct_n = cfg.direct_n;
    d.sm_n4 = std::max(0, std::min(cfg.small_n4, 16)); d.sm_n5 = std::max(d.sm_n4, std::min(cfg.small_n5, 32));
    if (!d.pos_packed || d.force_fft || !(p.gc_wei >= 0.0 && p.au_wei >= 0.0 && p.gu_wei >= 0.0)) d.sm_n4 = d.sm_n5 = 0;
    d.mat_tile = 64;
    d.mat_tile = std::max(1, std::min(cfg.mat_tile, 64));
    if (cfg.rl_cap >= 0) d.rl_cap = std::min(cfg.rl_cap, RL_CAP);
    d.beam = (int *)ws.beam.p; d.beam_n = (int *)ws.beam_n.p; d.done = (int *)ws.done.p; d.nsteps = (int *)ws.nsteps.p;
    d.ch_cap = c.ch_cap;
    d.ch_parent = (uint16_t *)ws.ch_parent.p; d.ch_combo = (uint64_t *)ws.ch_combo.p; d.ch_dcal = (int *)ws.ch_dcal.p; d.ch_h = (uint64_t *)ws.ch_h.p;
    d.seen = (uint64_t *)ws.seen.p; d.seen_cap_total = c.seen;
    d.seen_off = (uint64_t *)ws.seen_off.p; d.seen_cap = (uint32_t *)ws.seen_cap.p; d.seen_cnt = (uint32_t *)ws.seen_cnt.p;
    d.st_cap = (uint32_t)c.st;
    d.st = (StRec *)ws.st.p;
    d.prod = (ProdEnt *)ws.prod.p; d.prod_shard_cap = c.nd / NSHARD;
    d.nd_cap = (uint32_t)c.nd;
    d.nd = (NodeRec *)ws.nd.p; d.nlist = (int *)ws.nlist.p; d.nd_slot = (uint32_t *)ws.nd_slot.p; d.cslot = (unsigned long long *)ws.cslot.p;
    d.looptab = (unsigned long long *)ws.looptab.p; d.looptab_cap = c.looptab;
    d.pos = (uint16_t *)ws.pos.p; d.pos_cap = c.pos; d.br = (uint32_t *)ws.br.p; d.br_cap = c.br;
    d.sp = (uint32_t *)ws.sp.p; d.sp_cap = c.sp;
    d.cand = (Cand *)ws.cand.p; d.cand_cap = c.cand;
    d.trec = (int4 *)ws.trec.p; d.trec_cap = (uint32_t)c.trec; d.tsid = (int *)ws.tsid.p; d.tsid_cap = c.tsid;
    d.work[0] = (int *)ws.work0.p; d.work[1] = (int *)ws.work1.p; d.work[2] = (int *)ws.work2.p; d.work[3] = (int *)ws.work3.p;
    d.work[4] = (int *)ws.work4.p; d.work[5] = (int *)ws.work5.p; d.work_cap = (uint32_t)c.work;
    d.mat = (MatRec *)ws.mat.p; d.mat_cap = (uint32_t)c.mat;
    d.c = (Counters *)ws.counters.p;
    d.nd_base = S; d.nd_shard_cap = (c.nd - S) / NSHARD;
    d.pos_base = sumL; d.pos_shard_cap = (c.pos - sumL) / NSHARD;
    d.sp_shard_cap = c.sp / NSHARD;
    d.br_shard_cap = c.br / NSHARD; d.cand_shard_cap = c.cand / NSHARD;
    if (seam) d.dbg = seam->dbg;


    const double ms_plan = since(tw0);
    hipStream_t st = ws.stream;
    double t_mark = ms_plan;
    auto slow_call = [&](const char *what) {
        if (!cfg.trace) return;
        const double now = since(tw0);
        if (now - t_mark > 1.0) fprintf(stderr, "[rafft] setup of a wave of %zu sequences: %s kept the host for %.3f ms\n", S, what, now - t_mark);
        t_mark = now;
    };
    memset(&hc, 0, sizeof hc);
    hc.n_struct = S; hc.seen_top = seen0_total;
    memcpy((char *)stage.p + st_ctr, &hc, sizeof hc);
    {
        uint64_t *so = (uint64_t *)((char *)stage.p + st_soff);
        uint32_t *sc = (uint32_t *)((char *)stage.p + st_scap);
        size_t o = 0;
        for (size_t i = 0; i < S; i++) { so[i] = o; sc[i] = seen_cap0[i]; o += seen_cap0[i]; }
        StageIn si;
        memset(&si, 0, sizeof si);
        auto seg = [&](size_t off, void *dst, size_t bytes) {
            si.src[si.n] = (const uint32_t *)((const char *)stage.p + off); si.dst[si.n] = (uint32_t *)dst; si.words[si.n] = (bytes + 3) / 4; si.n++;
        };
        seg(st_codes, ws.codes.p, sumL + 16); seg(st_off, ws.seq_off.p, S * 4); seg(st_len, ws.seq_len.p, S * 4);
        seg(st_soff, ws.seen_off.p, S * 8); seg(st_scap, ws.seen_cap.p, S * 4); seg(st_ctr, ws.counters.p, sizeof hc);
        const size_t words = (sumL + 16 + 3) / 4;
        hipLaunchKernelGGL(stage_in_kernel, dim3((unsigned)std::min<size_t>((words + 255) / 256, 1024)), dim3(256), 0, st, si);
        HIPCHK(hipGetLastError());
    }
    slow_call("the launch of stage_in_kernel");
    if (d.memo) HIPCHK(hipMemsetAsync(ws.looptab.p, 0, c.looptab * 8, st));
    slow_call("the memset of the loop table");
    HIPCHK(hipMemsetAsync(ws.seen.p, 0, seen0_total * 16, st));
    slow_call("the memset of the seen tables");
    hipLaunchKernelGGL(init_roots_kernel, dim3((unsigned)S), dim3(64), 0, st, d);
    HIPCHK(hipGetLastError());
    slow_call("the launch of init_roots_kernel");
    if (seam) HIPCHK(hipStreamSynchronize(st));
    for (int v = 0; v < 2; v++) {
        const size_t nt = v ? 1024 : 256;
        bs_lds[v] = std::max((size_t)c.sort_cap * 8, 24 * nt) + RL_CAP * 12 + B * sizeof(ParentInfo) + (B + 1) * 8 + ((B + 3) & ~(size_t)3) * 4 + 128 + B * 4;
    }
    mat_lds = 20 * (size_t)d.max_prod;
    out_row_lds = ((size_t)maxL + 15) & ~(size_t)15;
    n_active = (unsigned)S;
    ms_setup = since(tw0);
    if (cfg.trace) fprintf(stderr, "[rafft] setup: encode %.3f ms, plan+buffers %.3f ms, copies+init %.3f ms\n", ms_enc, ms_plan - ms_enc, ms_setup - ms_plan);
    tw1 = std::chrono::steady_clock::now();
    return 0;
}

int Wave::issue_step()
{
    HostTimer acc_{ms_issue};
    hipStream_t st = ws.stream;
    const unsigned wide_below = (unsigned)std::max(0, cfg.wide_below);
    const bool serial = cfg.serial != 0;
    const unsigned small_wg_per_cu = (unsigned)std::max(1, cfg.small_wg);
    const size_t hot_len = offsetof(Counters, node);
    HIPCHK(hipEventRecord(ws.ev_fork, st));
    Span wall{next_event(), next_event(), 4};
    SPAN_REC(wall.a, st, 4);
    static const int order[NCLS] = {3, 0, 2, 1, 5, 4};
    for (int oi = 0; oi < NCLS; oi++) {
        const int cls = order[oi];
        if (cls == 0 && !longseq) continue;
        if (cls == 3 && merge_target == 2) continue;
        if (merged_now == 3 && cls != 3 && cls != 0) continue;
        if (merged_now == 2 && cls == 1) continue;
        if (cls >= NGEN && (merged_now != 0 || steps == 0 || (cls == 4 ? d.sm_n4 : d.sm_n5) == 0 || (cls == 5 && d.sm_n5 == d.sm_n4))) continue;
        const bool inline_ = serial || (merged_now == 3 && !longseq);
        hipStream_t cs = inline_ ? st : ws.cls_stream[cls];
        if (!inline_) HIPCHK(hipStreamWaitEvent(cs, ws.ev_fork, 0));
        Span sp{next_event(), next_event(), 10 + cls};
        SPAN_REC(sp.a, cs, sp.kind);
        unsigned grid = cls >= NGEN ? (unsigned)g.n_cu * small_wg_per_cu : (unsigned)cf[cls].grid;
        if (steps > 0) {
            const unsigned long long bound = (unsigned long long)last_mat * (cls == 1 ? 8ULL : 4ULL) + 32ULL;
            if (bound < grid) grid = (unsigned)bound;
        }
        if (int rc = launch_expand_cls(cfg, d, cls, cf, grid, cs)) return rc;
        if (cls == 1) bt.stats.n_expand_launches++;
        SPAN_REC(sp.b, cs, sp.kind);
        spans.push_back(sp);
        if (!inline_) {
            HIPCHK(hipEventRecord(ws.ev_join[cls], cs));
            HIPCHK(hipStreamWaitEvent(st, ws.ev_join[cls], 0));
        }
    }
    SPAN_REC(wall.b, st, 4);
    spans.push_back(wall);
    {
        Span sp{next_event(), next_event(), 1};
        SPAN_REC(sp.a, st, sp.kind);
        if (n_active < wide_below) hipLaunchKernelGGL((beam_step_kernel<1024>), dim3((unsigned)S), dim3(1024), bs_lds[1], st, d, c.sort_cap);
        else hipLaunchKernelGGL((beam_step_kernel<256>), dim3((unsigned)S), dim3(256), bs_lds[0], st, d, c.sort_cap);
        HIPCHK(hipGetLastError());
        SPAN_REC(sp.b, st, sp.kind);
        spans.push_back(sp);
    }
    steps++;
    HIPCHK(hipMemcpyAsync(ws.hot, ws.counters.p, hot_len, hipMemcpyDeviceToHost, st));
    HIPCHK(hipEventRecord(ws.ev_hot, st));
    t_issued = std::chrono::steady_clock::now();
    return 0;
}

int Wave::issue_materialize(unsigned nm)
{
    hipStream_t st = ws.stream;
    Span sp{next_event(), next_event(), 2};
    SPAN_REC(sp.a, st, sp.kind);
    if (d.max_prod <= MAT4_PROD)
        hipLaunchKernelGGL(materialize_team_kernel, dim3((nm + MAT4_TEAMS - 1) / MAT4_TEAMS), dim3(64), 0, st, d, (int)nm);
    else hipLaunchKernelGGL(materialize_kernel, dim3(nm), dim3(MAT_NT), mat_lds, st, d, (int)nm);
    HIPCHK(hipGetLastError());
    const unsigned merge_below = cfg.merge_below >= 0 ? (unsigned)cfg.merge_below : 2u * (unsigned)g.n_cu;
    const unsigned merge2_below = cfg.merge2_below >= 0 ? (unsigned)cfg.merge2_below : 128u * (unsigned)g.n_cu;
    d.merge_cls = seam ? 0 : nm < merge_below ? merge_target : nm < merge2_below ? 2 : 0;
    merged_now = d.merge_cls;
    const unsigned dd_grid = std::min<unsigned>((unsigned)g.n_cu * (1024u / DEDUPE_NT), (unsigned)std::min<unsigned long long>(0x7fffffffULL, (unsigned long long)nm * 4ULL / DEDUPE_NT + 2ULL));
    hipLaunchKernelGGL(dedupe_kernel, dim3(dd_grid), dim3(DEDUPE_NT), 0, st, d);
    HIPCHK(hipGetLastError());
    SPAN_REC(sp.b, st, sp.kind);
    spans.push_back(sp);
    return 0;
}

int Wave::after_beam()
{
    HostTimer acc_{ms_after};
    hipStream_t st = ws.stream;
    if (draining) return finish_done();
    const size_t hot_len = offsetof(Counters, node);
    memcpy(&hc, ws.hot, hot_len);
    if (hc.overflow) { ovf = hc.overflow; return finish(); }
    if (cfg.test_ovf_at >= 0 && depth == 0 && steps == cfg.test_ovf_at) { ovf = OVF_STRUCT; return finish(); }
    if (hc.n_mat == 0) return finish();
    n_active = (unsigned)S - hc.n_done;
    last_mat = hc.n_mat;
    const bool harvest_now = !p.traj && !seam && !harvested && S >= 256 && (size_t)hc.trec_n * 10 >= S * 7;
    const size_t harvest_n = (size_t)hc.trec_n;
    if (int rc = issue_materialize(hc.n_mat)) return rc;
    if (cfg.trace >= 2) {
        Counters h2;
        HIPCHK(hipMemcpyAsync(&h2, ws.counters.p, hot_len, hipMemcpyDeviceToHost, st));
        HIPCHK(hipStreamSynchronize(st));
        fprintf(stderr, "[rafft] step %d: n_mat %u -> work %u %u %u %u | small %u %u\n", steps, hc.n_mat, h2.n_work[0].v, h2.n_work[1].v, h2.n_work[2].v, h2.n_work[3].v, h2.n_work[4].v, h2.n_work[5].v);
    }
    const int step_of_harvest = steps;
    if (int rc = issue_step()) return rc;
    if (harvest_now && !finished) {
        if (int rc = emit_rows(0, harvest_n, true, nullptr)) return rc;
        harvested = harvest_n;
        if (cfg.trace) fprintf(stderr, "[rafft] early harvest after step %d: %zu of %zu sequences\n", step_of_harvest, harvested, S);
    }
    return 0;
}

int Wave::emit_rows(size_t first, size_t count, bool early, double *t_gather)
{
    const auto t0_ = std::chrono::steady_clock::now();
    hipStream_t st = early ? ws.copy_stream : ws.stream;
    Buf &b_rec = early ? ws.row_off2 : ws.row_off, &b_db = early ? ws.out_db2 : ws.out_db, &b_dc = early ? ws.out_dcal2 : ws.out_dcal;
    std::vector<int4> trec(count);
    if (count) HIPCHK(hipMemcpy(trec.data(), (const int4 *)ws.trec.p + first, count * sizeof(int4), hipMemcpyDeviceToHost));
    if (p.traj) std::sort(trec.begin(), trec.end(), [](const int4 &a, const int4 &b) { return a.x != b.x ? a.x < b.x : a.y < b.y; });
    std::vector<OutRec> &recs = early ? early_recs : late_recs;
    recs.assign(trec.size(), OutRec{});
    long long tot_bytes = 0;
    size_t nrows = 0;
    for (size_t ri = 0; ri < trec.size(); ri++) {
        const int4 &r = trec[ri];
        recs[ri] = OutRec{tot_bytes, (int)nrows, r.w, r.z, len[r.x]};
        tot_bytes += (long long)r.z * (len[r.x] + 1);
        nrows += (size_t)r.z;
    }
    if (t_gather) *t_gather = std::chrono::duration<double, std::milli>(std::chrono::steady_clock::now() - t0_).count();
    last_rows_bytes = tot_bytes;
    if (!nrows) return 0;
    const size_t dcal_off = ((size_t)tot_bytes + 63) & ~(size_t)63;
    PinBuf chunk;
    chunk = pin_acquire(dcal_off + nrows * 4 + 64);
    if (!chunk.p) return fail(RAFFT_ERR_HIP, "hipHostMalloc failed for the result buffer");
    {
        auto shared = std::make_shared<PinChunk>(chunk);
        for (auto &m : members) m->ho->chunks.push_back(shared);
    }
    char *all_db = (char *)chunk.p;
    int *all_dcal = (int *)((char *)chunk.p + dcal_off);
    if (int rc = ensure(b_rec, (size_t)((double)(recs.size() * sizeof(OutRec)) * reserve))) return rc;
    if (int rc = ensure(b_db, (size_t)((double)tot_bytes * reserve))) return rc;
    if (int rc = ensure(b_dc, (size_t)((double)(nrows * 4) * reserve))) return rc;
    HIPCHK(hipMemcpyAsync(b_rec.p, recs.data(), recs.size() * sizeof(OutRec), hipMemcpyHostToDevice, st));
    Span sp{next_event(), next_event(), 3};
    SPAN_REC(sp.a, st, sp.kind);
    unsigned grid = (unsigned)std::min<size_t>(nrows, 65536);
    hipLaunchKernelGGL(output_kernel, dim3(grid), dim3(64), out_row_lds, st, d, (int)nrows, (int)recs.size(), (const OutRec *)b_rec.p,
                       (char *)b_db.p, (int *)b_dc.p);
    HIPCHK(hipGetLastError());
    SPAN_REC(sp.b, st, sp.kind);
    spans.push_back(sp);
    HIPCHK(hipMemcpyAsync(all_db, b_db.p, (size_t)tot_bytes, hipMemcpyDeviceToHost, st));
    HIPCHK(hipMemcpyAsync(all_dcal, b_dc.p, nrows * 4, hipMemcpyDeviceToHost, st));
    for (size_t r0 = 0; r0 < recs.size();) {
        const int i = trec[r0].x;
        size_t r1 = r0;
        while (r1 < recs.size() && trec[r1].x == i) r1++;
        const int gi = seqs[i].idx;
        HostOut &out = out_of(i);
        int o = 0;
        if (r1 - r0 == 1) { out.one_size[gi] = o = recs[r0].cnt; out.one_off[gi] = 0; }
        else {
            auto &ss = out.step_size[gi];
            auto &so = out.step_off[gi];
            ss.resize(r1 - r0); so.resize(r1 - r0);
            for (size_t r = r0; r < r1; r++) { ss[r - r0] = recs[r].cnt; so[r - r0] = o; o += recs[r].cnt; }
        }
        out.dcal_ptr[gi] = all_dcal + recs[r0].row0;
        out.db_ptr[gi] = all_db + recs[r0].off;
        rafft_seq_result &sr = out.seq[gi];
        sr.status = RAFFT_OK; sr.length = len[i]; sr.n_steps = (int)(r1 - r0); sr.n_structs = o;
        r0 = r1;
    }
    return 0;
}

int Wave::finish_body()
{
    hipStream_t st = ws.stream;
    finished = true;
    tail.ms_loop = since(tw1);
    tail.t0 = std::chrono::steady_clock::now();
    bt.stats.n_steps = std::max<int64_t>(bt.stats.n_steps, steps);
    if (ovf && cfg.trace) fprintf(stderr, "[rafft] wave S=%zu est %.1f overflowed (bits %u) after %d steps, %.1f ms\n", S, est, ovf, steps, since(tw0));
    if (ovf) {
        HIPCHK(hipStreamSynchronize(st));
        if (harvested) HIPCHK(hipStreamSynchronize(ws.copy_stream));
        if ((ovf & OVF_PROD) && !(ovf & OVF_SORT) && d.max_prod < MAX_PROD_LONG) {
            want_big_prod = true;
            return result = RAFFT_ERR_CAPACITY;
        }
        if (ovf & (OVF_PROD | OVF_SORT))
            return result = fail(RAFFT_ERR_PARAM, "structure with more than 1024 productive regions, or sort capacity exceeded");
        return result = RAFFT_ERR_CAPACITY;
    }
    HIPCHK(hipMemcpy(&hc, ws.counters.p, sizeof hc, hipMemcpyDeviceToHost));
    for (int c = 0; c < NCLS; c++)
        for (int i = 0; i < NSHARD; i++) {
            const Counters::StatLine &x = hc.xstat[c][i];
            hc.n_expand += x.items; hc.sum_n += x.n; hc.sum_lags += x.lags; hc.sum_nbr += x.nbr;
            hc.cls_items[c] += x.items; hc.cls_sum_n[c] += x.n; hc.cls_sum_lags[c] += x.lags;
            hc.n_alias += x.alias; hc.n_children += x.children; hc.sum_struct_len += x.struct_len;
            bt.stats.n_dE_evals += (int64_t)x.evals; bt.stats.n_dE_guessed += (int64_t)x.guessed; bt.stats.n_kept_guessed += (int64_t)x.kept_guessed;
        }
    {
        unsigned long long nn = S, ni = S;
        for (int i = 0; i < NSHARD; i++) { nn += hc.node[i].v; ni += hc.nlist[i].v; }
        bt.stats.n_nodes_created += (int64_t)nn;
        bt.stats.n_node_instances += (int64_t)ni;
    }
    bt.stats.n_node_expansions += hc.n_expand;
    bt.stats.n_nodes_aliased += (int64_t)hc.n_alias;
    bt.stats.sum_node_len += hc.sum_n;
    bt.stats.sum_lags += hc.sum_lags;
    bt.stats.n_structs += (int64_t)hc.n_struct;
    bt.stats.n_children += hc.n_children;
    bt.stats.sum_struct_len += (int64_t)(hc.sum_struct_len + sumL);
    {
        int64_t ex = 3 * (int64_t)hc.sum_n + 16 * (int64_t)hc.sum_lags + 3 * (int64_t)(hc.sum_struct_len + sumL);
        double share = hc.n_expand ? (double)hc.cls_items[1] / (double)hc.n_expand : 0.0;
        bt.stats.alg_bytes_expand += 3 * (int64_t)hc.cls_sum_n[1] + 16 * (int64_t)hc.cls_sum_lags[1] +
                                    (int64_t)(share * 3.0 * (double)(hc.sum_struct_len + sumL));
        for (int c = 0; c < NCLS; c++) {
            const double sh = hc.n_expand ? (double)hc.cls_items[c] / (double)hc.n_expand : 0.0;
            const int64_t v = 3 * (int64_t)hc.cls_sum_n[c] + 16 * (int64_t)hc.cls_sum_lags[c] + (int64_t)(sh * 3.0 * (double)(hc.sum_struct_len + sumL));
            if (c == 2) bt.stats.alg_bytes_expand_c2 += v;
            else if (c == 3 || c == 0) bt.stats.alg_bytes_expand_c3 += v;
            else if (c >= NGEN) bt.stats.alg_bytes_expand_small += v;
        }
        bt.stats.alg_bytes_beam += 2 * (int64_t)hc.sum_struct_len + 8 * (int64_t)(hc.n_struct - S);
        bt.stats.alg_bytes_expand_all += ex;
        bt.stats.alg_bytes += ex + 2 * (int64_t)hc.sum_struct_len + 8 * (int64_t)(hc.n_struct - S);
    }


    tail.stats = since(tail.t0);
    if (int rc = emit_rows(harvested, (size_t)hc.trec_n - harvested, false, &tail.gather)) return rc;
    tail.gather += tail.stats;
    if (harvested) {
        HIPCHK(hipEventRecord(ws.ev_copy, ws.copy_stream));
        HIPCHK(hipStreamWaitEvent(st, ws.ev_copy, 0));
    }
    HIPCHK(hipEventRecord(ws.ev_hot, st));
    finished = false; draining = true;
    return 0;
}

int Wave::finish_done_body()
{
    finished = true;
    const double tl_copy = since(tail.t0);
    const long long tot_bytes = last_rows_bytes;
    if (cfg.trace) {
        auto mx = [&](const ShardCtr *sc) { unsigned long long m = 0, t = 0; for (int i = 0; i < NSHARD; i++) { m = std::max(m, sc[i].v); t += sc[i].v; } return std::make_pair(m, t); };
        auto nd = mx(hc.node), po = mx(hc.pos), br = mx(hc.br), spr = mx(hc.sp), ca = mx(hc.cand), pr = mx(hc.prod), nl = mx(hc.nlist);
        fprintf(stderr, "[rafft] max productive regions per structure: %u (limit %d)\n", hc.max_nprod, d.max_prod);
        fprintf(stderr, "[rafft] arenas used/cap (max shard | total): st %llu/%zu  nd %llu/%llu|%llu  pos %llu/%llu|%llu  br %llu/%llu|%llu  sp %llu/%llu|%llu  cand %llu/%llu|%llu  prod %llu/%llu|%llu  nlist %llu/%llu|%llu  seen %llu/%zu  est %.1f\n",
                hc.n_struct, c.st, nd.first, (unsigned long long)d.nd_shard_cap, nd.second, po.first, (unsigned long long)d.pos_shard_cap, po.second,
                br.first, (unsigned long long)d.br_shard_cap, br.second, spr.first, (unsigned long long)d.sp_shard_cap, spr.second,
                ca.first, (unsigned long long)d.cand_shard_cap, ca.second, pr.first, (unsigned long long)d.prod_shard_cap, pr.second, nl.first, (unsigned long long)d.nd_shard_cap, nl.second, hc.seen_top, c.seen, est);
    }
    if (cfg.trace >= 2) {
        std::vector<uint32_t> cnt(S), cap(S);
        HIPCHK(hipMemcpy(cnt.data(), d.seen_cnt, S * 4, hipMemcpyDeviceToHost));
        HIPCHK(hipMemcpy(cap.data(), d.seen_cap, S * 4, hipMemcpyDeviceToHost));
        const int edges[] = {0, 80, 100, 130, 200, 300, 500, 1000, 2000, 1 << 30};
        for (int e = 0; e + 1 < (int)(sizeof(edges) / sizeof(edges[0])); e++) {
            unsigned long long n = 0, sum = 0, mxc = 0, grown = 0, slots = 0;
            for (size_t i = 0; i < S; i++) if (len[i] > edges[e] && len[i] <= edges[e + 1]) { n++; sum += cnt[i]; mxc = std::max<unsigned long long>(mxc, cnt[i]); grown += cap[i] > seen_cap0[i] ? 1 : 0; slots += cap[i]; }
            if (n) fprintf(stderr, "[rafft] seen sets, %d < L <= %d: %llu sequences, mean %llu entries, max %llu, %llu grew, %llu slots at the end\n", edges[e], edges[e + 1], n, sum / n, mxc, grown, slots);
        }
    }
    if (cfg.trace) fprintf(stderr, "[rafft] host time inside issue_step %.3f ms, inside after_beam (incl. nested issue_step and this tail) %.3f ms\n", ms_issue, ms_after);
    if (cfg.trace) fprintf(stderr, "[rafft] wave S=%zu setup %.2f ms, loop %.2f ms (%d steps), tail %.2f ms (counters %.3f, records+gather %.3f, rows out %.3f incl. %.1f MB D2H)\n",
                                       S, ms_setup, tail.ms_loop, steps, since(tail.t0), tail.stats, tail.gather - tail.stats, tl_copy - tail.gather, (double)tot_bytes / 1e6);
    return result = 0;
}

int run_seam(Batch &bt, const std::vector<SeqIn> &one, const SeamIn &sm)
{
    Wave w(g.ws[0], {std::shared_ptr<Batch>(&bt, [](Batch *) {})}, one, 4.0, &sm);
    if (int rc = w.setup()) return rc;
    Workspace &W = g.ws[0];
    {
        std::vector<uint16_t> packed(sm.pos);
        if (w.d.pos_packed) {
            for (auto &v : packed) v = (uint16_t)(v | (kBaseCode[(unsigned char)one[0].s[v]] << 12));
        }
        HIPCHK(hipMemcpy(W.pos.p, packed.data(), packed.size() * 2, hipMemcpyHostToDevice));
    }
    if (!sm.br.empty()) {
        std::vector<uint32_t> pb(sm.br);
        if (w.d.pos_packed)
            for (auto &v : pb) v |= ((uint32_t)kBaseCode[(unsigned char)one[0].s[v & 0xFFFFu]] << 12) | ((uint32_t)kBaseCode[(unsigned char)one[0].s[v >> 16]] << 28);
        HIPCHK(hipMemcpy(W.br.p, pb.data(), pb.size() * 4, hipMemcpyHostToDevice));
    }
    int n = (int)sm.pos.size(), nbr = (int)sm.br.size();
    {
        NodeRec root;
        HIPCHK(hipMemcpy(&root, W.nd.p, sizeof root, hipMemcpyDeviceToHost));
        root.n = n; root.nbr = nbr; root.ci = sm.ci; root.cj = sm.cj; root.pdcal = sm.pdcal;
        HIPCHK(hipMemcpy(W.nd.p, &root, sizeof root, hipMemcpyHostToDevice));
    }
    int cls = node_class(n, (sm.ci < 0 || one[0].len > LDS_SEQ) ? one[0].len : sm.cj + 1 - sm.ci, nbr, 0, w.d.cls1_P, w.d.cls1_br, w.d.K, w.d.sm_n4, w.d.sm_n5);
    int zero = 0;
    memset(&w.hc.n_work, 0, sizeof w.hc.n_work);
    w.hc.n_work[cls].v = 1;
    HIPCHK(hipMemcpy(W.counters.p, &w.hc, sizeof w.hc, hipMemcpyHostToDevice));
    HIPCHK(hipMemcpy(w.d.work[cls], &zero, 4, hipMemcpyHostToDevice));
    if (int rc = launch_expand_cls(w.cfg, w.d, cls, w.cf, 1, W.stream)) return rc;
    HIPCHK(hipStreamSynchronize(W.stream));
    return 0;
}

}
```

Baseline: 541,300.

## Add LDS occupancy bitmap for seen hash tables to skip zeroing and empty-slot reads

Gives each small seen table an occupancy bitmap that is kept in LDS during the beam step and stored in global memory between steps. Lookups test the bitmap before reading 16-byte slots, inserts claim slots with an atomicOr on the bitmap, and setup only memsets the bitmap instead of the whole seen arena for bitmap-mode tables. This aims to cut global memory traffic for probing and table initialisation. In exchange it adds a bitmap load and store per step, larger LDS use that may lower occupancy of the 256-thread kernel, and a new failure path when a table outgrows the bitmap budget.

```diff
diff --git a/rafft_amd/csrc/rafft_beam.hip b/rafft_amd/csrc/rafft_beam.hip
--- a/rafft_amd/csrc/rafft_beam.hip
+++ b/rafft_amd/csrc/rafft_beam.hip
@@ -53,8 +53,43 @@
 }
 
 
+__device__ __forceinline__ bool bm_test(const uint32_t *bm, uint32_t s) { return (bm[s >> 5] >> (s & 31)) & 1u; }
+__device__ inline bool seen_lookup_bm(const uint64_t *tab, const uint32_t *bm, uint32_t cap, uint64_t h1, uint64_t h2, uint32_t &free_sl)
+{
+    const uint32_t mask = cap - 1;
+    uint32_t sl = (uint32_t)h1 & mask;
+    const ulonglong2 *t2 = (const ulonglong2 *)tab;
+    for (;;) {
+        if (!bm_test(bm, sl)) { free_sl = sl; return false; }
+        const uint32_t s1 = (sl + 1) & mask, s2 = (sl + 2) & mask, s3 = (sl + 3) & mask;
+        const bool b1 = bm_test(bm, s1), b2 = b1 && bm_test(bm, s2), b3 = b2 && bm_test(bm, s3);
+        ulonglong2 e0 = t2[sl], e1 = make_ulonglong2(0ULL, 0ULL), e2 = e1, e3 = e1;
+        if (b1) e1 = t2[s1];
+        if (b2) e2 = t2[s2];
+        if (b3) e3 = t2[s3];
+        pin(e0); pin(e1); pin(e2); pin(e3);
+        if (e0.x == h1 && e0.y == h2) return true;
+        if (!b1) { free_sl = s1; return false; }
+        if (e1.x == h1 && e1.y == h2) return true;
+        if (!b2) { free_sl = s2; return false; }
+        if (e2.x == h1 && e2.y == h2) return true;
+        if (!b3) { free_sl = s3; return false; }
+        if (e3.x == h1 && e3.y == h2) return true;
+        sl = (sl + 4) & mask;
+    }
+}
+__device__ inline void seen_insert_at_bm(uint64_t *tab, uint32_t *bm, uint32_t cap, uint64_t h1, uint64_t h2, uint32_t sl)
+{
+    const uint32_t mask = cap - 1;
+    for (;;) {
+        const uint32_t bit = 1u << (sl & 31);
+        if (!(atomicOr(&bm[sl >> 5], bit) & bit)) { ((ulonglong2 *)tab)[sl] = make_ulonglong2((unsigned long long)h1, (unsigned long long)h2); return; }
+        sl = (sl + 1) & mask;
+    }
+}
+
 template <int NT>
-__device__ inline void seen_rehash(const uint64_t *stab, uint32_t scap, uint64_t *ntab, uint32_t ncap, int tid)
+__device__ inline void seen_rehash(const uint64_t *stab, uint32_t scap, const uint32_t *sbm, uint64_t *ntab, uint32_t ncap, uint32_t *nbm, int tid)
 {
     const ulonglong2 *src = (const ulonglong2 *)stab;
     const uint32_t mask = ncap - 1;
@@ -62,7 +97,15 @@
         ulonglong2 e[4];
         unsigned long long old[4];
 #pragma unroll
-        for (int u = 0; u < 4; u++) { const uint32_t i = base + (uint32_t)u * NT + (uint32_t)tid; e[u] = i < scap ? src[i] : make_ulonglong2(0ULL, 0ULL); }
+        for (int u = 0; u < 4; u++) {
+            const uint32_t i = base + (uint32_t)u * NT + (uint32_t)tid;
+            e[u] = i < scap && (!sbm || bm_test(sbm, i)) ? src[i] : make_ulonglong2(0ULL, 0ULL);
+        }
+        if (nbm) {
+#pragma unroll
+            for (int u = 0; u < 4; u++) if (e[u].x) seen_insert_at_bm(ntab, nbm, ncap, e[u].x, e[u].y, (uint32_t)e[u].x & mask);
+            continue;
+        }
 #pragma unroll
         for (int u = 0; u < 4; u++) { old[u] = 1; if (e[u].x) old[u] = atomicCAS((unsigned long long *)&ntab[2 * (uint64_t)((uint32_t)e[u].x & mask)], 0ULL, (unsigned long long)e[u].x); }
 #pragma unroll
@@ -72,6 +115,40 @@
                 else seen_insert(ntab, ncap, e[u].x, e[u].y);
             }
     }
+}
+
+template <int NT>
+__device__ inline bool seen_grow(const Dev &d, int sq, uint32_t ncap, uint64_t *&stab, uint32_t &scap, bool &bmode, uint32_t *bm, uint32_t *obm,
+                                 uint32_t bm_max, int *sh, int tid)
+{
+    if (tid == 0) {
+        unsigned long long o = atomicAdd(&d.c->seen_top, (unsigned long long)ncap);
+        if (o + ncap > d.seen_cap_total || (o & 31)) { atomicOr(&d.c->overflow, OVF_SEEN); *(unsigned long long *)&sh[8] = ~0ULL; }
+        else *(unsigned long long *)&sh[8] = o;
+    }
+    __syncthreads();
+    const unsigned long long o = *(unsigned long long *)&sh[8];
+    __syncthreads();
+    if (o == ~0ULL) return false;
+    uint64_t *ntab = d.seen + 2 * o;
+    uint32_t t = (uint32_t)tid;
+    asm volatile("" : "+v"(t));
+    const bool nmode = ncap / 8 <= bm_max;
+    const uint32_t *sbm = bmode ? bm : nullptr;
+    if (bmode && nmode) {
+        for (uint32_t i = t; i < scap / 32; i += NT) obm[i] = bm[i];
+        sbm = obm;
+        __syncthreads();
+    }
+    if (nmode) for (uint32_t i = t; i < ncap / 32; i += NT) bm[i] = 0;
+    else for (uint32_t i = tid; i < ncap; i += NT) ((ulonglong2 *)ntab)[i] = make_ulonglong2(0ULL, 0ULL);
+    __syncthreads();
+    seen_rehash<NT>(stab, scap, sbm, ntab, ncap, nmode ? bm : nullptr, tid);
+    __syncthreads();
+    if (nmode) { uint32_t *gbm = d.seen_bm + o / 32; for (uint32_t i = t; i < ncap / 32; i += NT) gbm[i] = bm[i]; }
+    stab = ntab; scap = ncap; bmode = nmode;
+    if (tid == 0) { d.seen_off[sq] = o; d.seen_cap[sq] = ncap; d.seen_mode[sq] = nmode ? 1u : 0u; }
+    return true;
 }
 
 struct ParentInfo {
@@ -92,10 +169,10 @@
 }
 
 template <int BS_NT>
-__global__ __launch_bounds__(BS_NT, BS_NT == 256 ? 5 : 1) void beam_step_kernel(Dev d, int sort_cap)
+__global__ __launch_bounds__(BS_NT, BS_NT == 256 ? 5 : 1) void beam_step_kernel(Dev d, int sort_cap, int bm_max)
 {
     extern __shared__ __align__(16) unsigned char lds[];
-    const size_t r0 = max((size_t)8 * (size_t)sort_cap, (size_t)24 * BS_NT);
+    const size_t r0 = max((size_t)8 * (size_t)sort_cap, (size_t)24 * BS_NT + (size_t)bm_max);
     unsigned long long *skey = (unsigned long long *)lds;
     unsigned long long *wk_h1 = (unsigned long long *)lds;
     unsigned long long *wk_h2 = wk_h1 + BS_NT;
@@ -106,6 +183,8 @@
     unsigned long long *ppre = (unsigned long long *)(pinfo + d.B);
     int *oldbeam = (int *)(ppre + d.B + 1);
     int *sh = oldbeam + ((d.B + 3) & ~3);
+    uint32_t *bm = (uint32_t *)(lds + 24 * BS_NT);
+    uint32_t *obm = (uint32_t *)lds;
     const int tid = threadIdx.x, lane = tid & 63, wv = tid >> 6;
     const int sq = blockIdx.x;
     if (sq == 0 && tid < NSHARD) d.c->node_prev[tid].v = d.c->node[tid].v;
@@ -270,10 +349,22 @@
         }
         if (lane == 0) ppre[0] = 0;
     }
-    for (int i = tid; i < 2 * BS_NT; i += BS_NT) wk_tab[i] = 0;
-    __syncthreads();
     uint64_t *stab = d.seen + 2 * d.seen_off[sq];
     uint32_t scap = d.seen_cap[sq], scnt = d.seen_cnt[sq];
+    bool bmode = d.seen_mode[sq] != 0;
+    if (bmode && scap / 8 > (uint32_t)bm_max) {
+        if (tid == 0) atomicOr(&d.c->overflow, OVF_SEEN);
+        d.done[sq] = 1;
+        return;
+    }
+    if (bmode) {
+        const uint32_t *gbm = d.seen_bm + (size_t)(stab - d.seen) / 64;
+#pragma unroll 1
+        for (uint32_t i = tid; i < scap / 32; i += BS_NT) bm[i] = gbm[i];
+    }
+    bool seen_full = false;
+    for (int i = tid; i < 2 * BS_NT; i += BS_NT) wk_tab[i] = 0;
+    __syncthreads();
     const size_t chb = (size_t)sq * d.ch_cap;
     int nb_branch = 0, nchild = 0;
     int single_from = nbeam;
@@ -286,22 +377,7 @@
         if ((unsigned long long)(scnt + chunk) * 2 > scap) {
             uint32_t ncap = scap;
             while ((unsigned long long)(scnt + BS_NT) * 2 > ncap) ncap <<= 1;
-            if (tid == 0) {
-                unsigned long long o = atomicAdd(&d.c->seen_top, (unsigned long long)ncap);
-                if (o + ncap > d.seen_cap_total) { atomicOr(&d.c->overflow, OVF_SEEN); *(unsigned long long *)&sh[8] = ~0ULL; }
-                else *(unsigned long long *)&sh[8] = o;
-            }
-            __syncthreads();
-            unsigned long long o = *(unsigned long long *)&sh[8];
-            __syncthreads();
-            if (o == ~0ULL) { d.done[sq] = 1; return; }
-            uint64_t *ntab = d.seen + 2 * o;
-            for (uint32_t i = tid; i < ncap; i += BS_NT) ((ulonglong2 *)ntab)[i] = make_ulonglong2(0ULL, 0ULL);
-            __syncthreads();
-            seen_rehash<BS_NT>(stab, scap, ntab, ncap, tid);
-            __syncthreads();
-            stab = ntab; scap = ncap;
-            if (tid == 0) { d.seen_off[sq] = o; d.seen_cap[sq] = ncap; }
+            if (!seen_grow<BS_NT>(d, sq, ncap, stab, scap, bmode, bm, obm, (uint32_t)bm_max, sh, tid)) { seen_full = true; break; }
         }
         const int need = d.max_branch - nb_branch;
         int b = 0, sidb = 0, cd = 0, slot = -1;
@@ -365,7 +441,7 @@
             }
             h1 = a1 ? a1 : 1; h2 = a2 ? a2 : 1; cd = ad;
             wk_h1[tid] = h1; wk_h2[tid] = h2;
-            cand_new = !seen_lookup(stab, scap, h1, h2, free_sl);
+            cand_new = bmode ? !seen_lookup_bm(stab, bm, scap, h1, h2, free_sl) : !seen_lookup(stab, scap, h1, h2, free_sl);
         }
         if (cand_new) {
             unsigned int sl = (unsigned int)(h1 ^ (h1 >> 32)) & (2 * BS_NT - 1);
@@ -395,7 +471,8 @@
                 d.ch_h[2 * (chb + ci2)] = h1;
                 d.ch_h[2 * (chb + ci2) + 1] = h2;
             } else atomicOr(&d.c->overflow, OVF_SORT);
-            seen_insert_at(stab, scap, h1, h2, free_sl);
+            if (bmode) seen_insert_at_bm(stab, bm, scap, h1, h2, free_sl);
+            else seen_insert_at(stab, scap, h1, h2, free_sl);
         }
         if (hit) {
             if (accepted && ex == need - 1) {
@@ -416,29 +493,14 @@
         for (int i = tid; i < 2 * BS_NT; i += BS_NT) wk_tab[i] = 0;
         __syncthreads();
     }
-    if (single_from < nbeam) {
+    if (single_from < nbeam && !seen_full) {
         const int nrest = nbeam - single_from;
         if ((unsigned long long)(scnt + nrest) * 2 > scap) {
             uint32_t ncap = scap;
             while ((unsigned long long)(scnt + nrest + BS_NT) * 2 > ncap) ncap <<= 1;
-            if (tid == 0) {
-                unsigned long long o = atomicAdd(&d.c->seen_top, (unsigned long long)ncap);
-                if (o + ncap > d.seen_cap_total) { atomicOr(&d.c->overflow, OVF_SEEN); *(unsigned long long *)&sh[8] = ~0ULL; }
-                else *(unsigned long long *)&sh[8] = o;
-            }
-            __syncthreads();
-            unsigned long long o = *(unsigned long long *)&sh[8];
-            __syncthreads();
-            if (o == ~0ULL) { d.done[sq] = 1; return; }
-            uint64_t *ntab = d.seen + 2 * o;
-            for (uint32_t i = tid; i < ncap; i += BS_NT) ((ulonglong2 *)ntab)[i] = make_ulonglong2(0ULL, 0ULL);
-            __syncthreads();
-            seen_rehash<BS_NT>(stab, scap, ntab, ncap, tid);
-            __syncthreads();
-            stab = ntab; scap = ncap;
-            if (tid == 0) { d.seen_off[sq] = o; d.seen_cap[sq] = ncap; }
-        }
-        for (int base = single_from; base < nbeam; base += BS_NT) {
+            if (!seen_grow<BS_NT>(d, sq, ncap, stab, scap, bmode, bm, obm, (uint32_t)bm_max, sh, tid)) seen_full = true;
+        }
+        for (int base = single_from; base < nbeam && !seen_full; base += BS_NT) {
             const int b = base + tid;
             int isnew = 0;
             uint32_t free_sl = 0;
@@ -447,7 +509,7 @@
                 h1 = pinfo[b].h1; h2 = pinfo[b].h2;
                 if (h1 == 0) h1 = 1;
                 if (h2 == 0) h2 = 1;
-                isnew = seen_lookup(stab, scap, h1, h2, free_sl) ? 0 : 1;
+                isnew = (bmode ? seen_lookup_bm(stab, bm, scap, h1, h2, free_sl) : seen_lookup(stab, scap, h1, h2, free_sl)) ? 0 : 1;
                 for (int e = single_from; isnew && e < b; e++)
                     if (pinfo[e].flag == 0) {
                         uint64_t g1 = pinfo[e].h1, g2 = pinfo[e].h2;
@@ -466,13 +528,23 @@
                     d.ch_h[2 * (chb + ci2)] = h1;
                     d.ch_h[2 * (chb + ci2) + 1] = h2;
                 } else atomicOr(&d.c->overflow, OVF_SORT);
-                seen_insert_at(stab, scap, h1, h2, free_sl);
+                if (bmode) seen_insert_at_bm(stab, bm, scap, h1, h2, free_sl);
+                else seen_insert_at(stab, scap, h1, h2, free_sl);
             }
             if (b < nbeam && pinfo[b].flag == 0) { d.st[oldbeam[b]].cursor = 1; d.st[oldbeam[b]].total = pinfo[b].total; }
             nchild += tot; nb_branch += tot; scnt += tot;
             __syncthreads();
         }
     }
+    if (bmode) {
+        if (nchild > 0) {
+            uint32_t *gbm = d.seen_bm + (size_t)(stab - d.seen) / 64;
+#pragma unroll 1
+            for (uint32_t i = tid; i < scap / 32; i += BS_NT) gbm[i] = bm[i];
+        }
+        __syncthreads();
+    }
+    if (seen_full) { d.done[sq] = 1; return; }
     if (tid == 0) { d.seen_cnt[sq] = scnt; atomicAdd(&d.c->xstat[1][sq & (NSHARD - 1)].children, (unsigned long long)nchild); }
     if (nchild > d.ch_cap) nchild = d.ch_cap;
 
diff --git a/rafft_amd/csrc/rafft_config.h b/rafft_amd/csrc/rafft_config.h
--- a/rafft_amd/csrc/rafft_config.h
+++ b/rafft_amd/csrc/rafft_config.h
@@ -37,8 +37,10 @@
     int test_ovf_at = -1;
     int seen_fixed = 0;
     int test_cand_limit = 0;
+    int seen_bm_max = -1;
+    int pad_ = 0;
 };
-static_assert(sizeof(Config) == 8 * 6 + 4 * 30, "Config: 8-byte fields first, an even number of ints - no padding (same_config compares bytes)");
+static_assert(sizeof(Config) == 8 * 6 + 4 * 32, "Config: 8-byte fields first, an even number of ints - no padding (same_config compares bytes)");
 
 inline Config read_config()
 {
@@ -61,6 +63,7 @@
 #ifndef RAFFT_NO_TEST_HOOKS
     I("RAFFT_MAT_TILE", c.mat_tile); I("RAFFT_RL_CAP", c.rl_cap); F("RAFFT_EST", c.est); I("RAFFT_SEEN_FIXED", c.seen_fixed);
     I("RAFFT_TEST_CAND_LIMIT", c.test_cand_limit); I("RAFFT_TEST_HARD_FAIL", c.test_hard_fail); I("RAFFT_TEST_MAX_PROD", c.test_max_prod); I("RAFFT_TEST_OVF_AT", c.test_ovf_at);
+    I("RAFFT_SEEN_BM_MAX", c.seen_bm_max);
 #endif
     return c;
 }
diff --git a/rafft_amd/csrc/rafft_host_ctx.h b/rafft_amd/csrc/rafft_host_ctx.h
--- a/rafft_amd/csrc/rafft_host_ctx.h
+++ b/rafft_amd/csrc/rafft_host_ctx.h
@@ -25,7 +25,7 @@
 #define MAX_PIPES 4
 #define WS_BUFFERS(X)                                                                                                           \
     X(codes, 1) X(seq_off, 1) X(seq_len, 1) X(beam, 1) X(beam_n, 1) X(done, 1) X(nsteps, 1) X(ch_parent, 1) X(ch_combo, 1)      \
-    X(ch_dcal, 1) X(ch_h, 1) X(seen, 1) X(seen_off, 1) X(seen_cap, 1) X(seen_cnt, 1) X(st, 1) X(prod, 1) X(nd, 1) X(nlist, 1)   \
+    X(ch_dcal, 1) X(ch_h, 1) X(seen, 1) X(seen_off, 1) X(seen_cap, 1) X(seen_cnt, 1) X(seen_bm, 1) X(seen_mode, 1) X(st, 1) X(prod, 1) X(nd, 1) X(nlist, 1)   \
     X(nd_slot, 1) X(cslot, 1) X(pos, 1) X(br, 1) X(sp, 1) X(cand, 1) X(looptab, 1) X(trec, 1) X(tsid, 1) X(work0, 1)            \
     X(work1, 1) X(work2, 1) X(work3, 1) X(work4, 1) X(work5, 1) X(mat, 1) X(counters, 1) X(row_off, 1) X(out_db, 1)             \
     X(out_dcal, 1) X(row_off2, 1) X(out_db2, 1) X(out_dcal2, 1) X(dbg, 0) X(big, 0)
diff --git a/rafft_amd/csrc/rafft_io_kernels.hip b/rafft_amd/csrc/rafft_io_kernels.hip
--- a/rafft_amd/csrc/rafft_io_kernels.hip
+++ b/rafft_amd/csrc/rafft_io_kernels.hip
@@ -29,6 +29,7 @@
         d.beam[(size_t)sq * d.B] = sq; d.beam_n[sq] = 1; d.nsteps[sq] = 0;
         d.done[sq] = L > 0 ? 0 : 1;
         d.seen_cnt[sq] = 0;
+        d.seen_mode[sq] = d.seen_cap[sq] / 8 <= d.seen_bm0 ? 1u : 0u;
         if (L > 0) {
             int cls = node_class(L, L, 0, 0, d.cls1_P, d.cls1_br);
             unsigned int w = atomicAdd(&d.c->n_work[cls].v, 1u);
diff --git a/rafft_amd/csrc/rafft_kernels.h b/rafft_amd/csrc/rafft_kernels.h
--- a/rafft_amd/csrc/rafft_kernels.h
+++ b/rafft_amd/csrc/rafft_kernels.h
@@ -23,6 +23,7 @@
 #ifndef SEEN0
 #define SEEN0 8192
 #endif
+static_assert(SEEN0 >= 2048 && (SEEN0 & (SEEN0 - 1)) == 0, "seen tables are powers of two >= 2048 slots (their bitmaps start on whole words)");
 #define NCLS 6
 #define NGEN 4
 struct ShardCtr { unsigned long long v; unsigned long long pad[7]; };
@@ -95,6 +96,9 @@
     uint16_t *ch_parent; uint64_t *ch_combo; int *ch_dcal; uint64_t *ch_h;
     uint64_t *seen; uint64_t seen_cap_total;
     uint64_t *seen_off; uint32_t *seen_cap, *seen_cnt;
+    uint32_t *seen_bm;
+    uint32_t *seen_mode;
+    uint32_t seen_bm0;
     uint32_t st_cap;
     StRec *st;
     ProdEnt *prod; uint64_t prod_shard_cap;
diff --git a/rafft_amd/csrc/rafft_plan.h b/rafft_amd/csrc/rafft_plan.h
--- a/rafft_amd/csrc/rafft_plan.h
+++ b/rafft_amd/csrc/rafft_plan.h
@@ -171,7 +171,7 @@
     int need = p.max_branch + 2 * p.max_stack + 8;
     int m2 = 2; while (m2 < p.max_stack) m2 <<= 1;
     c.sort_cap = std::max((need + 1) & ~1, m2);
-    c.bytes = c.st * 128 + c.nd * (64 + 4 + 4 + 6 * 4 + 16) + c.pos * 2 + c.br * 4 + c.sp * 4 + c.cand * (32 + 8) + c.seen * 16 +
+    c.bytes = c.st * 128 + c.nd * (64 + 4 + 4 + 6 * 4 + 16) + c.pos * 2 + c.br * 4 + c.sp * 4 + c.cand * (32 + 8) + c.seen * 16 + c.seen / 8  +
               c.looptab * 8 + c.trec * 16 + c.tsid * 4 + c.mat * 48 + S * (size_t)c.ch_cap * 32 + S * B * 4;
     return c;
 }
diff --git a/rafft_amd/csrc/rafft_wave.h b/rafft_amd/csrc/rafft_wave.h
--- a/rafft_amd/csrc/rafft_wave.h
+++ b/rafft_amd/csrc/rafft_wave.h
@@ -73,12 +73,12 @@
     Batch &bt;
     std::vector<Span> &spans;
     const SeamIn *seam;
-    size_t S = 0, sumL = 0, B = 0, bs_lds[2] = {0, 0}, mat_lds = RAFFT_MAX_LEN, out_row_lds = RAFFT_MAX_LEN;
+    size_t S = 0, sumL = 0, B = 0, bs_lds[2] = {0, 0}, bs_bm[2] = {0, 0} , mat_lds = RAFFT_MAX_LEN, out_row_lds = RAFFT_MAX_LEN;
     double reserve = 1.0;
     bool longseq = false;
     std::vector<int> off, len;
     std::vector<uint32_t> seen_cap0;
-    size_t seen0_total = 0;
+    size_t seen0_total = 0, seen0_zeroed = 0;
     ClsCfg cf[NGEN + 1];
     Caps c;
     Dev d;
@@ -195,7 +195,7 @@
     ENS(codes, sumLr + 16); ENS(seq_off, Sr * 4); ENS(seq_len, Sr * 4);
     ENS(beam, Sr * B * 4); ENS(beam_n, Sr * 4); ENS(done, Sr * 4); ENS(nsteps, Sr * 4);
     ENS(ch_parent, Sr * c.ch_cap * 2); ENS(ch_combo, Sr * c.ch_cap * 8); ENS(ch_dcal, Sr * c.ch_cap * 4); ENS(ch_h, Sr * c.ch_cap * 16);
-    ENS(seen, cr.seen * 16); ENS(seen_off, Sr * 8); ENS(seen_cap, Sr * 4); ENS(seen_cnt, Sr * 4);
+    ENS(seen, cr.seen * 16); ENS(seen_off, Sr * 8); ENS(seen_cap, Sr * 4); ENS(seen_cnt, Sr * 4); ENS(seen_bm, cr.seen / 8 + 64); ENS(seen_mode, Sr * 4);
     ENS(st, cr.st * sizeof(StRec)); ENS(prod, cr.nd * 16);
     ENS(nd, cr.nd * sizeof(NodeRec)); ENS(nlist, cr.nd * 4); ENS(nd_slot, cr.nd * 4); ENS(cslot, cr.cand * 8);
     ENS(pos, cr.pos * 2); ENS(br, cr.br * 4); ENS(sp, cr.sp * 4); ENS(cand, cr.cand * 32);
@@ -245,6 +245,7 @@
     d.ch_parent = (uint16_t *)ws.ch_parent.p; d.ch_combo = (uint64_t *)ws.ch_combo.p; d.ch_dcal = (int *)ws.ch_dcal.p; d.ch_h = (uint64_t *)ws.ch_h.p;
     d.seen = (uint64_t *)ws.seen.p; d.seen_cap_total = c.seen;
     d.seen_off = (uint64_t *)ws.seen_off.p; d.seen_cap = (uint32_t *)ws.seen_cap.p; d.seen_cnt = (uint32_t *)ws.seen_cnt.p;
+    d.seen_bm = (uint32_t *)ws.seen_bm.p; d.seen_mode = (uint32_t *)ws.seen_mode.p;
     d.st_cap = (uint32_t)c.st;
     d.st = (StRec *)ws.st.p;
     d.prod = (ProdEnt *)ws.prod.p; d.prod_shard_cap = c.nd / NSHARD;
@@ -266,6 +267,18 @@
     if (seam) d.dbg = seam->dbg;
 
 
+    for (int v = 1; v >= 0; v--) {
+        const size_t nt = v ? 1024 : 256;
+        const size_t rest = RL_CAP * 12 + B * sizeof(ParentInfo) + (B + 1) * 8 + ((B + 3) & ~(size_t)3) * 4 + 128 + B * 4;
+        size_t bm = v ? 32768 : 4096;
+        if (cfg.seen_bm_max >= 0) bm = std::min((size_t)cfg.seen_bm_max & ~(size_t)15, 32 * nt);
+        while (bm && 24 * nt + bm + rest > 160 * 1024) bm = (bm / 2) & ~(size_t)15;
+        if (v == 0) bm = std::min(bm, bs_bm[1]);
+        bs_bm[v] = bm;
+        bs_lds[v] = std::max((size_t)c.sort_cap * 8, 24 * nt + bm) + rest;
+    }
+    d.seen_bm0 = (uint32_t)bs_bm[S < (size_t)std::max(0, cfg.wide_below) ? 1 : 0];
+
     const double ms_plan = since(tw0);
     hipStream_t st = ws.stream;
     double t_mark = ms_plan;
@@ -282,7 +295,14 @@
         uint64_t *so = (uint64_t *)((char *)stage.p + st_soff);
         uint32_t *sc = (uint32_t *)((char *)stage.p + st_scap);
         size_t o = 0;
-        for (size_t i = 0; i < S; i++) { so[i] = o; sc[i] = seen_cap0[i]; o += seen_cap0[i]; }
+        for (int big = 1; big >= 0; big--) {
+            for (size_t i = 0; i < S; i++) {
+                if ((seen_cap0[i] / 8 > d.seen_bm0) != (big != 0)) continue;
+                if ((o | seen_cap0[i]) & 31) return fail(RAFFT_ERR_PARAM, "internal: a seen table does not start on a whole word of the bitmap arena");
+                so[i] = o; sc[i] = seen_cap0[i]; o += seen_cap0[i];
+            }
+            if (big) seen0_zeroed = o;
+        }
         StageIn si;
         memset(&si, 0, sizeof si);
         auto seg = [&](size_t off, void *dst, size_t bytes) {
@@ -297,16 +317,13 @@
     slow_call("the launch of stage_in_kernel");
     if (d.memo) HIPCHK(hipMemsetAsync(ws.looptab.p, 0, c.looptab * 8, st));
     slow_call("the memset of the loop table");
-    HIPCHK(hipMemsetAsync(ws.seen.p, 0, seen0_total * 16, st));
-    slow_call("the memset of the seen tables");
+    if (d.seen_bm0) HIPCHK(hipMemsetAsync(ws.seen_bm.p, 0, seen0_total / 8, st));
+    if (seen0_zeroed) HIPCHK(hipMemsetAsync(ws.seen.p, 0, seen0_zeroed * 16, st));
+    slow_call("the memset of the seen bitmaps");
     hipLaunchKernelGGL(init_roots_kernel, dim3((unsigned)S), dim3(64), 0, st, d);
     HIPCHK(hipGetLastError());
     slow_call("the launch of init_roots_kernel");
     if (seam) HIPCHK(hipStreamSynchronize(st));
-    for (int v = 0; v < 2; v++) {
-        const size_t nt = v ? 1024 : 256;
-        bs_lds[v] = std::max((size_t)c.sort_cap * 8, 24 * nt) + RL_CAP * 12 + B * sizeof(ParentInfo) + (B + 1) * 8 + ((B + 3) & ~(size_t)3) * 4 + 128 + B * 4;
-    }
     mat_lds = 20 * (size_t)d.max_prod;
     out_row_lds = ((size_t)maxL + 15) & ~(size_t)15;
     n_active = (unsigned)S;
@@ -359,8 +376,8 @@
     {
         Span sp{next_event(), next_event(), 1};
         SPAN_REC(sp.a, st, sp.kind);
-        if (n_active < wide_below) hipLaunchKernelGGL((beam_step_kernel<1024>), dim3((unsigned)S), dim3(1024), bs_lds[1], st, d, c.sort_cap);
-        else hipLaunchKernelGGL((beam_step_kernel<256>), dim3((unsigned)S), dim3(256), bs_lds[0], st, d, c.sort_cap);
+        if (n_active < wide_below) hipLaunchKernelGGL((beam_step_kernel<1024>), dim3((unsigned)S), dim3(1024), bs_lds[1], st, d, c.sort_cap, (int)bs_bm[1]);
+        else hipLaunchKernelGGL((beam_step_kernel<256>), dim3((unsigned)S), dim3(256), bs_lds[0], st, d, c.sort_cap, (int)bs_bm[0]);
         HIPCHK(hipGetLastError());
         SPAN_REC(sp.b, st, sp.kind);
         spans.push_back(sp);
```

Result: faster. 564,200 (median of 6 runs) (+4.2%).
